# tub-rip/event_based_bos

Measured on AMD Instinct MI355X. Metric: Mevents/sec warped+IWE at 1280x720, higher is better.
Workload: dtype f32

## Files before the change

event_based_bos_amd/csrc/plan_lean.hip:

```cpp
#include <algorithm>
#include <type_traits>

#include "common.h"

namespace ebos {
namespace {

#ifdef EBOS_LEAN_STAMPS
__device__ unsigned long long g_lean_stamps[2][8192 * 8];
#define EBOS_LSTAMP(which, k)                                                                                     \
  do {                                                                                                            \
    if (threadIdx.x == 0 && blockIdx.x < 8192) g_lean_stamps[which][blockIdx.x * 8 + (k)] = wall_clock64();       \
  } while (0)
#else
#define EBOS_LSTAMP(which, k) \
  do {                        \
  } while (0)
#endif

constexpr int kChunk = 8192;
constexpr int kLeanBlock = 1024;
constexpr int kMaxBins = 8192;
constexpr int kSortBlock = 1024;
constexpr size_t kSortLds = 158 * 1024;

enum LeanSource { SRC_AOS_F32 = 0, SRC_AOS_F64 = 1, SRC_RAW32 = 2, SRC_RAW64 = 3 };

struct LeanIn {
  const void* events;
  const int16_t* col;
  const int16_t* row;
  const void* t;
  double ticks_per_second;
};

struct Ev {
  float x, y;
  double t;
};

template <int SRC>
__device__ __forceinline__ Ev read_event(const LeanIn& in, int64_t i) {
  Ev e;
  if (SRC == SRC_AOS_F32) {
    const float4 v = reinterpret_cast<const float4*>(in.events)[i];
    e.x = v.x, e.y = v.y, e.t = (double)v.z;
  } else if (SRC == SRC_AOS_F64) {
    const double2 a = reinterpret_cast<const double2*>(in.events)[2 * i];
    const double tt = reinterpret_cast<const double*>(in.events)[4 * i + 2];
    e.x = (float)a.x, e.y = (float)a.y, e.t = tt;
  } else {
    e.x = (float)in.row[i];
    e.y = (float)in.col[i];
    e.t = SRC == SRC_RAW32 ? (double)static_cast<const int32_t*>(in.t)[i] : (double)static_cast<const int64_t*>(in.t)[i];
  }
  return e;
}

struct LeanGeom {
  int H, W, th, tw, tiles_x, n_tiles, sub, n_bins;
  int chunk;
  unsigned m_th, m_tw;
};
__device__ __forceinline__ int div_small(int v, int d, unsigned m) { return m ? (int)__umulhi((unsigned)v, m) : v / d; }

__device__ __forceinline__ int event_bin(const LeanGeom& g, float x, float y, unsigned& pix, bool& fractional) {
  fractional = false;
  if (!(x > -1e9f && x < 1e9f && y > -1e9f && y < 1e9f)) return -1;
  const int r = (int)x, c = (int)y;
  if (r < 0 || r >= g.H || c < 0 || c >= g.W) return -1;
  fractional = (x != (float)r) || (y != (float)c) || x < 0.f || y < 0.f;
  const int ty = div_small(r, g.th, g.m_th), tx = div_small(c, g.tw, g.m_tw);
  const int rl = r - ty * g.th, cl = c - tx * g.tw;
  pix = ((unsigned)rl << 8) | (unsigned)cl;
  return (ty * g.tiles_x + tx) * g.sub + div_small(rl * g.sub, g.th, g.m_th);
}
__device__ __forceinline__ int band_row0(const LeanGeom& g, int s) { return (s * g.th + g.sub - 1) / g.sub; }

__device__ __forceinline__ unsigned long long ordered(double v) {
  const unsigned long long b = (unsigned long long)__double_as_longlong(v);
  return (b >> 63) ? ~b : (b | 0x8000000000000000ull);
}
__device__ __forceinline__ double unordered(unsigned long long u) {
  const unsigned long long b = (u >> 63) ? (u & 0x7fffffffffffffffull) : ~u;
  return __longlong_as_double((long long)b);
}

constexpr int kTabShift = 14;
constexpr unsigned kTabMask = (1u << kTabShift) - 1u;

struct ChunkPartial {
  double lo, hi;
  int bad, frac;
};

struct LeanScratch {
  unsigned* tab;
  int32_t* bin_base;
  unsigned long long* tm;
  unsigned* ticket;
  ChunkPartial* partial;
  uint16_t* stage_px;
  void* stage_t;
};

template <int SRC> struct StageT { typedef unsigned type; };
template <> struct StageT<SRC_AOS_F64> { typedef unsigned long long type; };
template <> struct StageT<SRC_RAW64> { typedef unsigned long long type; };

template <int SRC>
__device__ __forceinline__ typename StageT<SRC>::type read_stamp(const LeanIn& in, int64_t i, float& x, float& y, double& t) {
  if (SRC == SRC_AOS_F32) {
    const float4 v = reinterpret_cast<const float4*>(in.events)[i];
    x = v.x, y = v.y, t = (double)v.z;
    return (typename StageT<SRC>::type)__float_as_uint(v.z);
  } else if (SRC == SRC_AOS_F64) {
    const double2 a = reinterpret_cast<const double2*>(in.events)[2 * i];
    const double tt = reinterpret_cast<const double*>(in.events)[4 * i + 2];
    x = (float)a.x, y = (float)a.y, t = tt;
    return (typename StageT<SRC>::type)__double_as_longlong(tt);
  } else if (SRC == SRC_RAW32) {
    x = (float)in.row[i], y = (float)in.col[i];
    const int32_t k = static_cast<const int32_t*>(in.t)[i];
    t = (double)k;
    return (typename StageT<SRC>::type)(unsigned)k;
  } else {
    x = (float)in.row[i], y = (float)in.col[i];
    const int64_t k = static_cast<const int64_t*>(in.t)[i];
    t = (double)k;
    return (typename StageT<SRC>::type)k;
  }
}
__device__ __forceinline__ double stamp_seconds(int src, const void* stage_t, int64_t i, double ticks_per_second) {
  switch (src) {
    case SRC_AOS_F32: return (double)static_cast<const float*>(stage_t)[i];
    case SRC_AOS_F64: return static_cast<const double*>(stage_t)[i];
    case SRC_RAW32: return (double)static_cast<const int32_t*>(stage_t)[i] / ticks_per_second;
    default: return (double)static_cast<const int64_t*>(stage_t)[i] / ticks_per_second;
  }
}

__device__ __forceinline__ int32_t block_exclusive_scan(int32_t v, int32_t* s_wave , int32_t& total) {
  const int lane = threadIdx.x & (kWave - 1), wid = threadIdx.x / kWave;
  int32_t inc = v;
#pragma unroll
  for (int off = 1; off < kWave; off <<= 1) {
    const int32_t o = __shfl_up(inc, off, kWave);
    if (lane >= off) inc += o;
  }
  if (lane == kWave - 1) s_wave[wid] = inc;
  __syncthreads();
  int32_t wave_off = 0, tot = 0;
#pragma unroll
  for (int k = 0; k < kLeanBlock / kWave; ++k) {
    const int32_t w = s_wave[k];
    wave_off += k < wid ? w : 0;
    tot += w;
  }
  total = tot;
  __syncthreads();
  return wave_off + inc - v;
}

struct StageOne {
  LeanIn in;
  int64_t n;
  LeanGeom g;
  LeanScratch sc;
  struct View {
    LeanIn in;
    int64_t n;
    LeanGeom g;
    LeanScratch sc;
    __device__ __forceinline__ unsigned index() const { return blockIdx.x; }
    __device__ __forceinline__ unsigned count() const { return gridDim.x; }
  };
  __device__ __forceinline__ View view() const { return View{in, n, g, sc}; }
};

template <int SRC, typename Args>
__global__ void __launch_bounds__(kLeanBlock, 8)
lean_stage_kernel(Args args) {
  const typename Args::View v = args.view();
  const LeanIn in = v.in;
  const int64_t n = v.n;
  const LeanGeom g = v.g;
  const LeanScratch sc = v.sc;
  typedef typename StageT<SRC>::type stamp_t;
  extern __shared__ int32_t s_mem[];
  int32_t* s_hist = s_mem;
  stamp_t* s_t = reinterpret_cast<stamp_t*>(s_mem + ((g.n_bins + 1) & ~1));
  uint16_t* s_px = reinterpret_cast<uint16_t*>(s_t + g.chunk);
  __shared__ int32_t s_wave[kLeanBlock / kWave + 1];
  EBOS_LSTAMP(0, 0);
  for (int b = threadIdx.x; b < g.n_bins; b += kLeanBlock) s_hist[b] = 0;
  if (v.index() == 0 && threadIdx.x == 0) *sc.ticket = 0u;
  __syncthreads();
  constexpr int kPer = kChunk / kLeanBlock;
  const int64_t base = (int64_t)v.index() * g.chunk;
  const int64_t chunk_end = min(n, base + g.chunk);
  double lo = 1.0e308 * 10.0, hi = -1.0e308 * 10.0;
  int bad = 0, frac = 0;
  int bin_of[kPer];
  unsigned pix[kPer];
  stamp_t stamp[kPer];
#pragma unroll
  for (int k = 0; k < kPer; ++k) {
    if (k == kPer / 2) asm volatile("" ::: "memory");
    const int64_t i = base + k * kLeanBlock + threadIdx.x;
    bin_of[k] = -1;
    if (i < chunk_end) {
      float x, y;
      double t;
      stamp[k] = read_stamp<SRC>(in, i, x, y, t);
      lo = t < lo ? t : lo;
      hi = t > hi ? t : hi;
      bool fr;
      const int b = event_bin(g, x, y, pix[k], fr);
      bin_of[k] = b;
      bad += b < 0;
      frac += fr;
    }
  }
  EBOS_LSTAMP(0, 1);
#pragma unroll
  for (int k = 0; k < kPer; ++k)
    if (bin_of[k] >= 0) bin_of[k] |= atomicAdd(&s_hist[bin_of[k]], 1) << 13;
  __syncthreads();
  EBOS_LSTAMP(0, 2);
  const int per = (g.n_bins + kLeanBlock - 1) / kLeanBlock;
  const int b0 = threadIdx.x * per;
  int32_t mine = 0;
  for (int j = 0; j < per; ++j) mine += b0 + j < g.n_bins ? s_hist[b0 + j] : 0;
  int32_t kept;
  int32_t run = block_exclusive_scan(mine, s_wave, kept);
  for (int j = 0; j < per; ++j)
    if (b0 + j < g.n_bins) {
      const int32_t c = s_hist[b0 + j];
      s_hist[b0 + j] = run;
      sc.tab[(int64_t)(b0 + j) * v.count() + v.index()] = (unsigned)run | ((unsigned)c << kTabShift);
      run += c;
    }
  __syncthreads();
  EBOS_LSTAMP(0, 3);
#pragma unroll
  for (int k = 0; k < kPer; ++k)
    if (bin_of[k] >= 0) {
      const int pos = s_hist[bin_of[k] & 8191] + (bin_of[k] >> 13);
      s_t[pos] = stamp[k];
      s_px[pos] = (uint16_t)pix[k];
    }
  __syncthreads();
  EBOS_LSTAMP(0, 4);
  stamp_t* out_t = static_cast<stamp_t*>(sc.stage_t) + base;
  for (int i = threadIdx.x; i < kept; i += kLeanBlock) out_t[i] = s_t[i];
  unsigned* out_px = reinterpret_cast<unsigned*>(sc.stage_px + base);
  const unsigned* s_px2 = reinterpret_cast<const unsigned*>(s_px);
  for (int i = threadIdx.x; i < (kept + 1) / 2; i += kLeanBlock) out_px[i] = s_px2[i];
  __shared__ double s_lo[kLeanBlock / kWave], s_hi[kLeanBlock / kWave];
  __shared__ int s_bad[kLeanBlock / kWave], s_frac[kLeanBlock / kWave];
  lo = wave_min(lo);
  hi = wave_max(hi);
  bad = wave_sum(bad);
  frac = wave_sum(frac);
  if ((threadIdx.x & (kWave - 1)) == 0) {
    s_lo[threadIdx.x / kWave] = lo;
    s_hi[threadIdx.x / kWave] = hi;
    s_bad[threadIdx.x / kWave] = bad;
    s_frac[threadIdx.x / kWave] = frac;
  }
  __syncthreads();
  if (threadIdx.x == 0) {
    for (int k = 1; k < kLeanBlock / kWave; ++k) {
      lo = s_lo[k] < lo ? s_lo[k] : lo;
      hi = s_hi[k] > hi ? s_hi[k] : hi;
      bad += s_bad[k];
      frac += s_frac[k];
    }
    sc.partial[v.index()] = ChunkPartial{lo, hi, bad, frac};
  }
  EBOS_LSTAMP(0, 5);
}

struct WholeGrid {
  __device__ __forceinline__ unsigned index() const { return blockIdx.x; }
  __device__ __forceinline__ unsigned count() const { return gridDim.x; }
};
struct GridPart {
  unsigned idx, cnt;
  __device__ __forceinline__ unsigned index() const { return idx; }
  __device__ __forceinline__ unsigned count() const { return cnt; }
};

__device__ __forceinline__ void lean_scan_bins_block(const LeanGeom& g, const LeanScratch& sc, int32_t* __restrict__ grp_offsets,
                                                     int32_t* __restrict__ key_offsets, int64_t n_keys, double ticks_per_second, int raw,
                                                     double* __restrict__ tminmax) {
  __shared__ int32_t s_wave[1024 / kWave];
  __shared__ int32_t s_carry;
  typedef __attribute__((address_space(1))) int32_t gi32_;
  auto total_of = [&](int b) { return __hip_atomic_load((gi32_*)(sc.bin_base + b), __ATOMIC_RELAXED, __HIP_MEMORY_SCOPE_AGENT); };
  const int lane = threadIdx.x & (kWave - 1), wid = threadIdx.x / kWave;
  auto scan = [&](int count, auto value, auto store) {
    if (threadIdx.x == 0) s_carry = 0;
    __syncthreads();
    for (int start = 0; start < count; start += 1024) {
      const int i = start + threadIdx.x;
      const int32_t v = i < count ? value(i) : 0;
      int32_t inc = v;
#pragma unroll
      for (int off = 1; off < kWave; off <<= 1) {
        const int32_t o = __shfl_up(inc, off, kWave);
        if (lane >= off) inc += o;
      }
      if (lane == kWave - 1) s_wave[wid] = inc;
      __syncthreads();
      int32_t wave_off = 0;
      for (int k = 0; k < wid; ++k) wave_off += s_wave[k];
      const int32_t carry = s_carry;
      if (i < count) store(i, carry + wave_off + inc - v);
      __syncthreads();
      if (threadIdx.x == 1023) s_carry = carry + wave_off + inc;
      __syncthreads();
    }
  };
  scan(g.n_tiles,
       [&](int t) {
         int32_t c = 0;
         for (int s = 0; s < g.sub; ++s) c += total_of(t * g.sub + s);
         return (c + 3) >> 2;
       },
       [&](int t, int32_t pre) { grp_offsets[t] = pre; });
  if (threadIdx.x == 0) grp_offsets[g.n_tiles] = s_carry;
  __syncthreads();
  scan(g.n_bins, [&](int b) { return total_of(b); }, [&](int b, int32_t pre) { sc.bin_base[b] = pre; });
  if (threadIdx.x == 0) {
    sc.bin_base[g.n_bins] = s_carry;
    key_offsets[n_keys] = s_carry;
    if (tminmax != nullptr) {
      const double lo = unordered(sc.tm[0]), hi = unordered(sc.tm[1]);
      tminmax[0] = raw ? lo / ticks_per_second : lo;
      tminmax[1] = raw ? hi / ticks_per_second : hi;
    }
  }
}

template <typename Grid>
__device__ __forceinline__ void lean_totals_body(const LeanGeom& g, int n_chunks, const LeanScratch& sc, int32_t* __restrict__ counts,
                                                 int32_t* __restrict__ grp_offsets, int32_t* __restrict__ key_offsets, int64_t n_keys,
                                                 double ticks_per_second, int raw, double* __restrict__ tminmax, const Grid grid) {
  __shared__ int s_is_last;
  {
    const int bin = grid.index() * (kLeanBlock / kWave) + (int)(threadIdx.x / kWave), lane = threadIdx.x & (kWave - 1);
    if (bin < g.n_bins) {
      const unsigned* __restrict__ row = sc.tab + (int64_t)bin * n_chunks;
      int32_t acc = 0;
      constexpr int kU = 4;
      for (int c = lane; c < n_chunks; c += kWave * kU) {
        unsigned v[kU];
#pragma unroll
        for (int u = 0; u < kU; ++u) v[u] = c + kWave * u < n_chunks ? row[c + kWave * u] : 0u;
#pragma unroll
        for (int u = 0; u < kU; ++u) acc += (int32_t)(v[u] >> kTabShift);
      }
      acc = wave_sum(acc);
      if (lane == 0) {
        typedef __attribute__((address_space(1))) int32_t gi32_;
        __hip_atomic_store((gi32_*)(sc.bin_base + bin), acc, __ATOMIC_RELAXED, __HIP_MEMORY_SCOPE_AGENT);
        asm volatile("s_waitcnt vmcnt(0)" ::: "memory");
      }
    }
  }
  if (grid.index() == 0) {
    double lo = 1.0e308 * 10.0, hi = -1.0e308 * 10.0;
    int bad = 0, frac = 0;
    for (int c = threadIdx.x; c < n_chunks; c += kLeanBlock) {
      const ChunkPartial p = sc.partial[c];
      lo = p.lo < lo ? p.lo : lo;
      hi = p.hi > hi ? p.hi : hi;
      bad += p.bad;
      frac += p.frac;
    }
    __shared__ double s_lo[kLeanBlock / kWave], s_hi[kLeanBlock / kWave];
    __shared__ int s_bad[kLeanBlock / kWave], s_frac[kLeanBlock / kWave];
    lo = wave_min(lo);
    hi = wave_max(hi);
    bad = wave_sum(bad);
    frac = wave_sum(frac);
    if ((threadIdx.x & (kWave - 1)) == 0) {
      s_lo[threadIdx.x / kWave] = lo;
      s_hi[threadIdx.x / kWave] = hi;
      s_bad[threadIdx.x / kWave] = bad;
      s_frac[threadIdx.x / kWave] = frac;
    }
    __syncthreads();
    if (threadIdx.x == 0) {
      for (int k = 1; k < kLeanBlock / kWave; ++k) {
        lo = s_lo[k] < lo ? s_lo[k] : lo;
        hi = s_hi[k] > hi ? s_hi[k] : hi;
        bad += s_bad[k];
        frac += s_frac[k];
      }
      typedef __attribute__((address_space(1))) unsigned long long gu64_;
      __hip_atomic_store((gu64_*)&sc.tm[0], lo <= hi ? ordered(lo) : ~0ull, __ATOMIC_RELAXED, __HIP_MEMORY_SCOPE_AGENT);
      __hip_atomic_store((gu64_*)&sc.tm[1], lo <= hi ? ordered(hi) : 0ull, __ATOMIC_RELAXED, __HIP_MEMORY_SCOPE_AGENT);
      counts[0] = bad;
      counts[1] = frac;
    }
  }
  __syncthreads();
  if (threadIdx.x == 0) {
    typedef __attribute__((address_space(1))) unsigned gu32_;
    asm volatile("s_waitcnt vmcnt(0)" ::: "memory");
    const unsigned n_wg = grid.count();
    s_is_last = __hip_atomic_fetch_add((gu32_*)sc.ticket, 1u, __ATOMIC_RELAXED, __HIP_MEMORY_SCOPE_AGENT) == n_wg - 1u;
  }
  __syncthreads();
  if (!s_is_last) return;
  if (threadIdx.x == 0) {
    typedef __attribute__((address_space(1))) unsigned long long gu64_;
    sc.tm[0] = __hip_atomic_load((gu64_*)&sc.tm[0], __ATOMIC_RELAXED, __HIP_MEMORY_SCOPE_AGENT);
    sc.tm[1] = __hip_atomic_load((gu64_*)&sc.tm[1], __ATOMIC_RELAXED, __HIP_MEMORY_SCOPE_AGENT);
  }
  __syncthreads();
  lean_scan_bins_block(g, sc, grp_offsets, key_offsets, n_keys, ticks_per_second, raw, tminmax);
}

__global__ void __launch_bounds__(kLeanBlock)
lean_totals_kernel(LeanGeom g, int n_chunks, LeanScratch sc, int32_t* __restrict__ counts, int32_t* __restrict__ grp_offsets,
                   int32_t* __restrict__ key_offsets, int64_t n_keys, double ticks_per_second, int raw, double* __restrict__ tminmax) {
  lean_totals_body(g, n_chunks, sc, counts, grp_offsets, key_offsets, n_keys, ticks_per_second, raw, tminmax, WholeGrid{});
}

struct LeanTime {
  int src, ref_mode, normalize_t;
  double ref_fraction, ticks_per_second;
};

template <int STRIDE>
__device__ __forceinline__ int row_xor(int v) {
  static_assert(STRIDE == 1 || STRIDE == 2 || STRIDE == 4 || STRIDE == 8, "row_xor: 1, 2, 4 or 8");
  if (STRIDE == 1) return __builtin_amdgcn_update_dpp(0, v, 0xB1, 0xf, 0xf, false);
  if (STRIDE == 2) return __builtin_amdgcn_update_dpp(0, v, 0x4E, 0xf, 0xf, false);
  if (STRIDE == 8) return __builtin_amdgcn_update_dpp(0, v, 0x128, 0xf, 0xf, false);
  const int m = __builtin_amdgcn_update_dpp(0, v, 0x141, 0xf, 0xf, false);
  return __builtin_amdgcn_update_dpp(0, m, 0x1B, 0xf, 0xf, false);
}
template <int SIZE, int STRIDE>
__device__ __forceinline__ int bitonic16_step(int key, int sub16) {
  const int other = row_xor<STRIDE>(key);
  const bool up = (sub16 & SIZE) == 0;
  const bool low = (sub16 & STRIDE) == 0;
  const int mn = min(key, other), mx = max(key, other);
  return (low == up) ? mn : mx;
}
__device__ __forceinline__ int bitonic16(int key, int sub16, int longest) {
  key = bitonic16_step<2, 1>(key, sub16);
  if (longest > 2) {
    key = bitonic16_step<4, 2>(key, sub16);
    key = bitonic16_step<4, 1>(key, sub16);
  }
  if (longest > 4) {
    key = bitonic16_step<8, 4>(key, sub16);
    key = bitonic16_step<8, 2>(key, sub16);
    key = bitonic16_step<8, 1>(key, sub16);
  }
  if (longest > 8) {
    key = bitonic16_step<16, 8>(key, sub16);
    key = bitonic16_step<16, 4>(key, sub16);
    key = bitonic16_step<16, 2>(key, sub16);
    key = bitonic16_step<16, 1>(key, sub16);
  }
  return key;
}

__device__ __forceinline__ int sort_key(float d) {
  const int b = __float_as_int(d);
  return b ^ ((b >> 31) & 0x7fffffff);
}

struct LeanRec {
  unsigned pix;
  unsigned long long stamp;
};
struct LeanClock {
  double ref, inv_period, tps;
  bool raw, wide;
  __device__ __forceinline__ LeanClock(const LeanScratch& sc, const LeanTime& tc) {
    raw = tc.src == SRC_RAW32 || tc.src == SRC_RAW64;
    wide = tc.src == SRC_AOS_F64 || tc.src == SRC_RAW64;
    tps = tc.ticks_per_second;
    double tmin = unordered(sc.tm[0]), tmax = unordered(sc.tm[1]);
    if (raw) {
      tmin = tmin / tps;
      tmax = tmax / tps;
    } else if (tc.src == SRC_AOS_F32) {
      tmin = (double)(float)tmin;
      tmax = (double)(float)tmax;
    }
    if (tc.ref_mode == EBOS_REF_FIRST) ref = tmin;
    else if (tc.ref_mode == EBOS_REF_LAST) ref = tmax;
    else ref = tmin + (tmax - tmin) * tc.ref_fraction;
    inv_period = tc.normalize_t ? 1.0 / (tmax - tmin) : 1.0;
  }
  __device__ __forceinline__ float dt(const LeanRec& r) const {
    const double t8 = raw ? (double)(long long)r.stamp / tps : __longlong_as_double((long long)r.stamp);
    const double t4 = raw ? (double)(int32_t)(unsigned)r.stamp / tps : (double)__uint_as_float((unsigned)r.stamp);
    return (float)(((wide ? t8 : t4) - ref) * inv_period);
  }
};

template <bool POS, int BLOCK, typename Load, typename Use>
__device__ __forceinline__ void lean_gather(const LeanScratch& sc, const LeanGeom& g, int bin, int n_chunks, int32_t* s_arrived, Load&& load,
                                            Use&& use) {
  typedef decltype(load((int64_t)0)) payload_t;
  const int lane = threadIdx.x & (kWave - 1);
  const unsigned* __restrict__ my_tab = sc.tab + (int64_t)bin * n_chunks;
  unsigned e_next = (int)threadIdx.x < n_chunks ? my_tab[threadIdx.x] : 0u;
  for (int blk = 0; blk < n_chunks; blk += BLOCK) {
    const unsigned e = e_next;
    const int c_next = blk + BLOCK + threadIdx.x;
    e_next = c_next < n_chunks ? my_tab[c_next] : 0u;
    const int my_cnt = (int)(e >> kTabShift), my_off = (int)(e & kTabMask);
    if (__ballot(my_cnt > 0) == 0ull) continue;
    int my_pos = 0;
    if (POS) {
      int inc = my_cnt;
#pragma unroll
      for (int off = 1; off < kWave; off <<= 1) {
        const int o = __shfl_up(inc, off, kWave);
        if (lane >= off) inc += o;
      }
      int wave_base = 0;
      if (lane == kWave - 1) wave_base = atomicAdd(s_arrived, inc);
      my_pos = __shfl(wave_base, kWave - 1, kWave) + inc - my_cnt;
    }
    const int64_t wave_chunk0 = blk + (threadIdx.x & ~(kWave - 1));
    const int i0 = lane & 7;
    for (int base = 0; __ballot(my_cnt > base) != 0ull; base += 16) {
      payload_t v[16];
      int cnt[8], pos[8];
#pragma unroll
      for (int k = 0; k < 8; ++k) {
        const int r = 8 * k + (lane >> 3);
        cnt[k] = __shfl(my_cnt, r, kWave) - base;
        pos[k] = (POS ? __shfl(my_pos, r, kWave) : 0) + base;
        const int off = __shfl(my_off, r, kWave);
        const int64_t src = cnt[k] > 0 ? (wave_chunk0 + r) * g.chunk + off + base : 0;
        v[2 * k] = load(src + min(i0, max(cnt[k] - 1, 0)));
        v[2 * k + 1] = load(src + min(i0 + 8, max(cnt[k] - 1, 0)));
      }
#pragma unroll
      for (int k = 0; k < 8; ++k) {
        if (i0 < cnt[k]) use(v[2 * k], pos[k] + i0);
        if (i0 + 8 < cnt[k]) use(v[2 * k + 1], pos[k] + i0 + 8);
      }
    }
  }
}

__device__ __forceinline__ void lean_bin_sort_body(const LeanGeom& g, const LeanScratch& sc, const int32_t* __restrict__ grp_offsets,
                                                   int32_t* __restrict__ key_offsets, uint16_t* __restrict__ cpix, float* __restrict__ cdt,
                                                   int pix_cap, int sort_cap, int n_chunks, const LeanTime& tc) {
  extern __shared__ int32_t s_raw[];
  int32_t* s_cnt = s_raw;
  int32_t* s_cur = s_raw + pix_cap;
  float* a_dt = reinterpret_cast<float*>(s_raw + 2 * pix_cap);
  float* s_dt = a_dt + sort_cap;
  uint16_t* a_px = reinterpret_cast<uint16_t*>(s_dt + sort_cap);
  uint16_t* s_px = a_px + sort_cap;
  __shared__ int32_t s_wave[kSortBlock / kWave];
  __shared__ int32_t s_arrived;
  const int per_xcd = (g.n_bins + 7) / 8;
  const int bin = (int)(blockIdx.x & 7u) * per_xcd + (int)(blockIdx.x >> 3);
  if (bin >= g.n_bins) return;
  const int tile = bin / g.sub, band = bin - tile * g.sub;
  const int r0 = band_row0(g, band), r1 = band_row0(g, band + 1);
  const int n_pix = (r1 - r0) * g.tw;
  const int32_t seg0 = sc.bin_base[bin], seg1 = sc.bin_base[bin + 1], len = seg1 - seg0;
  const int64_t first_key = (int64_t)tile * g.th * g.tw + (int64_t)r0 * g.tw;
  const int32_t tile_first = sc.bin_base[tile * g.sub];
  const int64_t out0 = (int64_t)grp_offsets[tile] * 4 + (seg0 - tile_first);
  EBOS_LSTAMP(1, 0);
  for (int i = threadIdx.x; i < n_pix; i += kSortBlock) s_cnt[i] = 0;
  if (threadIdx.x == 0) s_arrived = 0;
  __syncthreads();
  const bool staged = len <= sort_cap;
  const int lane = threadIdx.x & (kWave - 1);
  const LeanClock clock(sc, tc);
  typedef LeanRec Rec;
  auto dt_of = [&](const Rec& r) { return clock.dt(r); };
  const bool wide = clock.wide;
  auto load8 = [&](int64_t i) { return Rec{(unsigned)sc.stage_px[i], static_cast<const unsigned long long*>(sc.stage_t)[i]}; };
  auto load4 = [&](int64_t i) { return Rec{(unsigned)sc.stage_px[i], (unsigned long long)static_cast<const unsigned*>(sc.stage_t)[i]}; };
  auto for_each_staged = [&](auto with_pos, auto&& load, auto&& use) {
    lean_gather<decltype(with_pos)::value, kSortBlock>(sc, g, bin, n_chunks, &s_arrived, load, use);
  };
  if (staged) {
    auto arrive = [&](const Rec& r, int at) {
      a_px[at] = (uint16_t)r.pix;
      a_dt[at] = dt_of(r);
      atomicAdd(&s_cnt[((int)(r.pix >> 8) - r0) * g.tw + (int)(r.pix & 255u)], 1);
    };
    if (wide) for_each_staged(std::true_type{}, load8, arrive);
    else for_each_staged(std::true_type{}, load4, arrive);
  } else {
    for_each_staged(std::false_type{}, [&](int64_t i) { return (unsigned)sc.stage_px[i]; },
                    [&](unsigned pix, int) { atomicAdd(&s_cnt[((int)(pix >> 8) - r0) * g.tw + (int)(pix & 255u)], 1); });
  }
  __syncthreads();
  EBOS_LSTAMP(1, 1);
  const int wid = threadIdx.x / kWave;
  {
    const int per = (n_pix + kSortBlock - 1) / kSortBlock, p0 = threadIdx.x * per;
    int32_t mine = 0;
    for (int j = 0; j < per; ++j) mine += p0 + j < n_pix ? s_cnt[p0 + j] : 0;
    int32_t inc = mine;
#pragma unroll
    for (int off = 1; off < kWave; off <<= 1) {
      const int32_t o = __shfl_up(inc, off, kWave);
      if (lane >= off) inc += o;
    }
    if (lane == kWave - 1) s_wave[wid] = inc;
    __syncthreads();
    int32_t run = inc - mine;
    for (int k = 0; k < wid; ++k) run += s_wave[k];
    for (int j = 0; j < per; ++j)
      if (p0 + j < n_pix) {
        const int32_t c = s_cnt[p0 + j];
        s_cnt[p0 + j] = run;
        s_cur[p0 + j] = run;
        key_offsets[first_key + p0 + j] = seg0 + run;
        run += c;
      }
    __syncthreads();
  }
  EBOS_LSTAMP(1, 2);
  if (staged) {
    for (int i = threadIdx.x; i < len; i += kSortBlock) {
      const unsigned pix = (unsigned)a_px[i];
      const int32_t pos = atomicAdd(&s_cur[((int)(pix >> 8) - r0) * g.tw + (int)(pix & 255u)], 1);
      s_px[pos] = (uint16_t)pix;
      s_dt[pos] = a_dt[i];
    }
  }
  __syncthreads();
  EBOS_LSTAMP(1, 3);
  if (!staged) {
    s_dt = a_dt;
    s_px = a_px;
    sort_cap *= 2;
  }
  constexpr int kLeanCanon = 1024, kHotList = 32;
  __shared__ int32_t s_hot[kHotList];
  __shared__ int32_t s_nhot, s_nlong;
  auto run_end = [&](int pi) { return pi + 1 < n_pix ? s_cnt[pi + 1] : len; };
  int p_lo = 0;
  while (p_lo < n_pix) {
    const int c0 = s_cnt[p_lo];
    int p_hi = n_pix;
    if (!staged) {
      int lo = p_lo, hi = n_pix;
      while (lo < hi) {
        const int mid = lo + (hi - lo) / 2;
        if (run_end(mid) - c0 <= sort_cap) lo = mid + 1;
        else hi = mid;
      }
      p_hi = lo;
    }
    const bool direct = p_hi == p_lo;
    if (direct) p_hi = p_lo + 1;
    const int c1 = p_hi < n_pix ? s_cnt[p_hi] : len, m = c1 - c0;
    if (threadIdx.x == 0) s_nhot = 0, s_nlong = 0;
    if (!staged) {
      __syncthreads();
      auto keep = [&](const Rec& r, int) {
        const int pi = ((int)(r.pix >> 8) - r0) * g.tw + (int)(r.pix & 255u);
        if (pi >= p_lo && pi < p_hi) {
          const int32_t pos = atomicAdd(&s_cur[pi], 1);
          if (direct) {
            cpix[out0 + pos] = (uint16_t)r.pix;
            cdt[out0 + pos] = dt_of(r);
          } else {
            s_px[pos - c0] = (uint16_t)r.pix;
            s_dt[pos - c0] = dt_of(r);
          }
        }
      };
      if (wide) for_each_staged(std::false_type{}, load8, keep);
      else for_each_staged(std::false_type{}, load4, keep);
      if (direct) {
        p_lo = p_hi;
        continue;
      }
    }
    __syncthreads();
    for (int pi = p_lo + threadIdx.x; pi < p_hi; pi += kSortBlock)
      if (run_end(pi) - s_cnt[pi] > kLeanCanon) {
        const int k = atomicAdd(&s_nhot, 1);
        if (k < kHotList) s_hot[k] = pi;
      }
    __syncthreads();
    EBOS_LSTAMP(1, 5);
    for (int i = threadIdx.x; i < m; i += kSortBlock) cpix[out0 + c0 + i] = s_px[i];
    const int n_hot = min(s_nhot, kHotList);
    for (int h = 0; h < n_hot; ++h) {
      const int pi = s_hot[h];
      const int rb = s_cnt[pi] - c0, L = run_end(pi) - c0 - rb;
      float* v = s_dt + rb;
      int n2 = 1;
      while (n2 < L) n2 <<= 1;
      for (int size = 2; size <= n2; size <<= 1) {
        for (int stride = size >> 1; stride > 0; stride >>= 1) {
          for (int t = threadIdx.x; t < n2 / 2; t += kSortBlock) {
            const int blk = t / stride, off = t - blk * stride, lo = blk * 2 * stride + off;
            const int hi = stride == (size >> 1) ? blk * 2 * stride + (2 * stride - 1 - off) : lo + stride;
            if (hi < L) {
              const float x = v[lo], y = v[hi];
              if (sort_key(x) > sort_key(y)) v[lo] = y, v[hi] = x;
            }
          }
          __syncthreads();
        }
      }
    }
    EBOS_LSTAMP(1, 6);
    const bool sparse = m < 4 * (p_hi - p_lo);
    if (sparse) {
      for (int i = threadIdx.x; i < m; i += kSortBlock) {
        const unsigned px = (unsigned)s_px[i];
        const int pi = ((int)(px >> 8) - r0) * g.tw + (int)(px & 255u);
        const int rb = s_cnt[pi] - c0, re = run_end(pi) - c0;
        const float d = s_dt[i];
        int slot = i;
        if (re - rb > 1 && re - rb <= kLeanCanon) {
          const int kd = sort_key(d);
          int rank = 0;
          for (int j = rb; j < re; ++j) {
            const int kj = sort_key(s_dt[j]);
            rank += (kj < kd || (kj == kd && j < i)) ? 1 : 0;
          }
          slot = rb + rank;
        }
        cdt[out0 + c0 + slot] = d;
      }
    } else {
      const int sub16 = lane & 15;
      for (int p0 = p_lo; p0 < p_hi; p0 += kSortBlock / 16) {
        const int pi = p0 + (threadIdx.x >> 4);
        const bool live = pi < p_hi;
        const int rb = live ? s_cnt[pi] - c0 : 0, L = live ? run_end(pi) - c0 - rb : 0;
        const bool small = L <= 16;
        int key = small && sub16 < L ? sort_key(s_dt[rb + sub16]) : 0x7fffffff;
        const int longest = __ballot(small && L > 8) != 0ull ? 16 : (__ballot(small && L > 4) != 0ull ? 8 : (__ballot(small && L > 2) != 0ull ? 4 : (__ballot(small && L > 1) != 0ull ? 2 : 1)));
        if (longest > 1) key = bitonic16(key, sub16, longest);
        if (small && sub16 < L) cdt[out0 + c0 + rb + sub16] = __int_as_float(key ^ ((key >> 31) & 0x7fffffff));
        if (!small && sub16 == 0) s_cur[atomicAdd(&s_nlong, 1)] = pi;
      }
    }
    __syncthreads();
    if (!sparse) {
      const int n_long = s_nlong, sub32 = lane & 31;
      for (int q = threadIdx.x >> 5; q < n_long; q += kSortBlock / 32) {
        const int pi = s_cur[q];
        const int rb = s_cnt[pi] - c0, L = run_end(pi) - c0 - rb;
        for (int e = sub32; e < L; e += 32) {
          const float d = s_dt[rb + e];
          int slot = e;
          if (L <= kLeanCanon) {
            const int kd = sort_key(d);
            int rank = 0;
            for (int j = 0; j < L; ++j) {
              const int kj = sort_key(s_dt[rb + j]);
              rank += (kj < kd || (kj == kd && j < e)) ? 1 : 0;
            }
            slot = rank;
          }
          cdt[out0 + c0 + rb + slot] = d;
        }
      }
    }
    EBOS_LSTAMP(1, 7);
    __syncthreads();
    p_lo = p_hi;
  }
  EBOS_LSTAMP(1, 4);
  if (band == g.sub - 1) {
    const int64_t end = (int64_t)grp_offsets[tile + 1] * 4;
    for (int64_t o = out0 + len + threadIdx.x; o < end; o += kSortBlock) {
      cpix[o] = 0;
      cdt[o] = __builtin_nanf("");
    }
  }
}

__global__ void __launch_bounds__(kSortBlock)
lean_bin_sort_kernel(LeanGeom g, LeanScratch sc, const int32_t* __restrict__ grp_offsets, int32_t* __restrict__ key_offsets,
                     uint16_t* __restrict__ cpix, float* __restrict__ cdt, int pix_cap, int sort_cap, int n_chunks, LeanTime tc) {
  lean_bin_sort_body(g, sc, grp_offsets, key_offsets, cpix, cdt, pix_cap, sort_cap, n_chunks, tc);
}

struct LeanSections {
  size_t off_base, off_tm, off_partial, off_px, off_t, total;
};
__host__ __device__ __forceinline__ LeanSections lean_sections(int n_bins, int n_chunks, int chunk) {
  auto align = [](size_t v) { return (v + 255) & ~(size_t)255; };
  LeanSections S;
  S.off_base = align((size_t)n_bins * n_chunks * 4);
  S.off_tm = S.off_base + align((size_t)(n_bins + 1) * 4);
  S.off_partial = S.off_tm + 256;
  S.off_px = S.off_partial + align((size_t)n_chunks * sizeof(ChunkPartial));
  S.off_t = S.off_px + align((size_t)n_chunks * chunk * 2);
  S.total = S.off_t + align((size_t)n_chunks * chunk * 8);
  return S;
}
__host__ __device__ __forceinline__ LeanScratch lean_scratch_at(char* base, const LeanSections& S) {
  return LeanScratch{reinterpret_cast<unsigned*>(base), reinterpret_cast<int32_t*>(base + S.off_base),
                     reinterpret_cast<unsigned long long*>(base + S.off_tm), reinterpret_cast<unsigned*>(base + S.off_tm + 64),
                     reinterpret_cast<ChunkPartial*>(base + S.off_partial), reinterpret_cast<uint16_t*>(base + S.off_px),
                     base + S.off_t};
}
__host__ __device__ __forceinline__ void lean_sort_caps(int th, int tw, int sub, int& pix_cap, int& sort_cap) {
  pix_cap = ((th + sub - 1) / sub + 1) * tw;
  const long long room = (long long)kSortLds - (long long)pix_cap * 8;
  sort_cap = room > 0 ? (int)(room / 12) & ~1 : 0;
}

struct LeanLayout {
  int n_chunks, chunk, sub, n_bins, pix_cap, sort_cap;
  size_t off_base, off_tm, off_partial, off_px, off_t, total;
};

inline LeanLayout lean_layout(int64_t n, int H, int W, int th, int tw) {
  LeanLayout L;
  const int n_tiles = ((H + th - 1) / th) * ((W + tw - 1) / tw);
  constexpr int64_t kResident = 512;
  int64_t c = (n + kChunk - 1) / kChunk;
  if (c > kResident) c = (c + kResident - 1) / kResident * kResident;
  else c = std::min<int64_t>(kResident, std::max<int64_t>(1, (n + kLeanBlock - 1) / kLeanBlock));
  L.chunk = (int)(((std::max<int64_t>(n, 1) + c - 1) / c + 7) & ~(int64_t)7);
  L.n_chunks = (int)((std::max<int64_t>(n, 1) + L.chunk - 1) / L.chunk);
  constexpr double kBinFill = 3.3;
  for (int sub = 1;; sub *= 2) {
    if (sub > th) sub = th;
    L.sub = sub;
    lean_sort_caps(th, tw, sub, L.pix_cap, L.sort_cap);
    if (sub == th || ((double)n / ((double)n_tiles * sub) <= kBinFill * L.sort_cap)) break;
  }
  L.n_bins = n_tiles * L.sub;
  const LeanSections S = lean_sections(L.n_bins, L.n_chunks, L.chunk);
  L.off_base = S.off_base, L.off_tm = S.off_tm, L.off_partial = S.off_partial, L.off_px = S.off_px, L.off_t = S.off_t, L.total = S.total;
  return L;
}

struct LeanWin {
  int64_t begin;
  int64_t scratch_off;
  int64_t slot_off;
  int32_t n;
  int32_t chunk0;
  int32_t n_chunks, chunk, sub;
  int32_t reserved;
};
constexpr int kLeanBatch = 64;
struct LeanBatch {
  LeanWin w[kLeanBatch];
};
static_assert(sizeof(LeanBatch) <= 3072, "the batch travels in the kernel argument segment");
struct LeanBatchOut {
  int32_t* key_offsets;
  int32_t* grp_offsets;
  uint16_t* cpix;
  float* cdt;
  int32_t* counts;
  double* tminmax;
  char* scratch;
  int64_t key_stride, grp_stride;
  int first;
};
__device__ __forceinline__ LeanIn lean_window_in(const LeanIn& in, int wide, int64_t begin) {
  return LeanIn{nullptr, in.col + begin, in.row + begin,
                wide ? static_cast<const void*>(static_cast<const int64_t*>(in.t) + begin)
                     : static_cast<const void*>(static_cast<const int32_t*>(in.t) + begin),
                in.ticks_per_second};
}
__device__ __forceinline__ LeanGeom lean_window_geom(LeanGeom g, const LeanWin& w) {
  g.sub = w.sub, g.n_bins = g.n_tiles * w.sub, g.chunk = w.chunk;
  return g;
}
__device__ __forceinline__ LeanScratch lean_window_scratch(const LeanBatchOut& o, const LeanGeom& g, const LeanWin& w) {
  return lean_scratch_at(o.scratch + w.scratch_off, lean_sections(g.n_bins, w.n_chunks, w.chunk));
}

struct StageMany {
  LeanBatch b;
  int n_windows, wide;
  LeanIn in;
  LeanGeom g0;
  LeanBatchOut o;
  struct View {
    LeanIn in;
    int64_t n;
    LeanGeom g;
    LeanScratch sc;
    unsigned idx, cnt;
    __device__ __forceinline__ unsigned index() const { return idx; }
    __device__ __forceinline__ unsigned count() const { return cnt; }
  };
  __device__ __forceinline__ View view() const {
    int lo = 0, hi = n_windows - 1;
    while (lo < hi) {
      const int mid = (lo + hi + 1) >> 1;
      if ((unsigned)b.w[mid].chunk0 <= blockIdx.x) lo = mid;
      else hi = mid - 1;
    }
    const LeanWin w = b.w[lo];
    const LeanGeom g = lean_window_geom(g0, w);
    return View{lean_window_in(in, wide, w.begin), (int64_t)w.n, g, lean_window_scratch(o, g, w), blockIdx.x - (unsigned)w.chunk0,
                (unsigned)w.n_chunks};
  }
};
static_assert(sizeof(StageMany) <= 3584, "the batch travels in the kernel argument segment");

__global__ void __launch_bounds__(kLeanBlock)
lean_totals_batch_kernel(LeanBatch b, LeanGeom g0, LeanBatchOut o, int64_t n_keys, double ticks_per_second) {
  const LeanWin w = b.w[blockIdx.y];
  const LeanGeom g = lean_window_geom(g0, w);
  const unsigned n_wg = (unsigned)((g.n_bins + kLeanBlock / kWave - 1) / (kLeanBlock / kWave));
  if (blockIdx.x >= n_wg) return;
  const int64_t wi = o.first + (int64_t)blockIdx.y;
  lean_totals_body(g, w.n_chunks, lean_window_scratch(o, g, w), o.counts + 2 * wi, o.grp_offsets + wi * o.grp_stride,
                   o.key_offsets + wi * o.key_stride, n_keys, ticks_per_second, 1, o.tminmax ? o.tminmax + 2 * wi : nullptr,
                   GridPart{blockIdx.x, n_wg});
}

__global__ void __launch_bounds__(kSortBlock)
lean_bin_sort_batch_kernel(LeanBatch b, LeanGeom g0, LeanBatchOut o, LeanTime tc) {
  const LeanWin w = b.w[blockIdx.y];
  const LeanGeom g = lean_window_geom(g0, w);
  if (blockIdx.x >= 8u * (unsigned)((g.n_bins + 7) / 8)) return;
  const int64_t wi = o.first + (int64_t)blockIdx.y;
  int pix_cap, sort_cap;
  lean_sort_caps(g.th, g.tw, g.sub, pix_cap, sort_cap);
  lean_bin_sort_body(g, lean_window_scratch(o, g, w), o.grp_offsets + wi * o.grp_stride, o.key_offsets + wi * o.key_stride,
                     o.cpix + w.slot_off, o.cdt + w.slot_off, pix_cap, sort_cap, w.n_chunks, tc);
}

}
}

extern "C" {

#ifdef EBOS_LEAN_STAMPS
int ebos_debug_read_lean_stamps(unsigned long long* host, int count) {
  return (int)hipMemcpyFromSymbol(host, HIP_SYMBOL(ebos::g_lean_stamps), sizeof(unsigned long long) * count);
}
#endif

size_t ebos_plan_lean_scratch_bytes(int64_t n, int H, int W, int tile_h, int tile_w) {
  if (n < 0 || H <= 0 || W <= 0 || tile_h <= 0 || tile_w <= 0) return 0;
  return ebos::lean_layout(n, H, W, tile_h, tile_w).total;
}

int ebos_plan_lean(int source, const void* events, const int16_t* col, const int16_t* row, const void* t, double ticks_per_second,
                   int64_t n, int ref_mode, double ref_fraction, int normalize_t, int H, int W, int tile_h, int tile_w,
                   int32_t* key_offsets, int32_t* grp_offsets, uint16_t* cpix, float* cdt, int64_t capacity_slots, int32_t* counts,
                   double* tminmax, void* scratch, size_t scratch_bytes, ebos_stream_t stream) {
  using namespace ebos;
  EBOS_REQUIRE(source >= 0 && source <= 3, "ebos_plan_lean: source must be 0 (f32 [n,4]), 1 (f64 [n,4]), 2 (raw, int32 t), 3 (raw, int64 t)");
  EBOS_REQUIRE(n >= 1 && n < (int64_t)1 << 31, "ebos_plan_lean: 1 <= n < 2^31 (got %lld)", (long long)n);
  EBOS_REQUIRE(H > 0 && W > 0 && tile_h > 0 && tile_w > 0 && tile_h <= 256 && tile_w <= 256, "ebos_plan_lean: bad sizes (tiles up to 256 x 256)");
  EBOS_REQUIRE(ref_mode >= 0 && ref_mode <= 2, "ebos_plan_lean: ref_mode must be FIRST / LAST / FRACTION");
  EBOS_REQUIRE(source <= 1 ? events != nullptr : (col && row && t && ticks_per_second > 0.0), "ebos_plan_lean: NULL event buffer");
  EBOS_REQUIRE(key_offsets && grp_offsets && cpix && cdt && counts && scratch, "ebos_plan_lean: NULL output / scratch");
  const int tiles_y = (H + tile_h - 1) / tile_h, tiles_x = (W + tile_w - 1) / tile_w, n_tiles = tiles_y * tiles_x;
  const int64_t n_keys = (int64_t)n_tiles * tile_h * tile_w;
  const LeanLayout L = lean_layout(n, H, W, tile_h, tile_w);
  if (L.n_bins > kMaxBins || L.sort_cap < 64) {
    set_error("ebos_plan_lean: %d bins / %d pixels per band exceed what this build sorts in LDS", L.n_bins, L.pix_cap);
    return EBOS_ERR_UNSUPPORTED;
  }
  if (scratch_bytes < L.total) {
    set_error("ebos_plan_lean: scratch too small (%zu < %zu)", scratch_bytes, L.total);
    return EBOS_ERR_SCRATCH;
  }
  if (capacity_slots < n + 3 * (int64_t)n_tiles + 4) {
    set_error("ebos_plan_lean: capacity %lld < n + 3 tiles + 4 = %lld", (long long)capacity_slots, (long long)(n + 3 * (int64_t)n_tiles + 4));
    return EBOS_ERR_SCRATCH;
  }
  hipStream_t s = as_stream(stream);
  char* base = reinterpret_cast<char*>(scratch);
  const LeanScratch sc = lean_scratch_at(base, lean_sections(L.n_bins, L.n_chunks, L.chunk));
  const bool small = H <= 65536 && W <= 65536;
  const LeanGeom g{H, W, tile_h, tile_w, tiles_x, n_tiles, L.sub, L.n_bins, L.chunk,
                   small ? (unsigned)(0x100000000ull / (unsigned)tile_h) + 1u : 0u, small ? (unsigned)(0x100000000ull / (unsigned)tile_w) + 1u : 0u};
  const LeanIn in{events, col, row, t, ticks_per_second};
  const size_t stamp_bytes = (source == SRC_AOS_F64 || source == SRC_RAW64) ? 8 : 4;
  const size_t lds_stage = (size_t)((L.n_bins + 1) & ~1) * 4 + (size_t)L.chunk * (stamp_bytes + 2);
  const size_t lds_sort = (size_t)(2 * L.pix_cap) * 4 + (size_t)L.sort_cap * 12;
  bool ok = hipFuncSetAttribute(reinterpret_cast<const void*>(lean_bin_sort_kernel), hipFuncAttributeMaxDynamicSharedMemorySize,
                                (int)kSortLds) == hipSuccess;
#define EBOS_LEAN_ATTR(SRC)                                                                                                  \
  ok = ok && hipFuncSetAttribute(reinterpret_cast<const void*>(lean_stage_kernel<SRC, StageOne>), hipFuncAttributeMaxDynamicSharedMemorySize, \
                                 (int)lds_stage) == hipSuccess
#define EBOS_LEAN(SRC)                                                                                                       \
  do {                                                                                                                       \
    EBOS_LEAN_ATTR(SRC);                                                                                                     \
    if (ok) lean_stage_kernel<SRC, StageOne><<<dim3(L.n_chunks), dim3(kLeanBlock), lds_stage, s>>>(StageOne{in, n, g, sc});  \
  } while (0)
  if (source == SRC_AOS_F32) EBOS_LEAN(SRC_AOS_F32);
  else if (source == SRC_AOS_F64) EBOS_LEAN(SRC_AOS_F64);
  else if (source == SRC_RAW32) EBOS_LEAN(SRC_RAW32);
  else EBOS_LEAN(SRC_RAW64);
#undef EBOS_LEAN
#undef EBOS_LEAN_ATTR
  if (!ok) {
    set_error("ebos_plan_lean: cannot reserve LDS for the staging pass / the bin sort");
    return EBOS_ERR_LAUNCH;
  }
  lean_totals_kernel<<<dim3((L.n_bins + kLeanBlock / kWave - 1) / (kLeanBlock / kWave)), dim3(kLeanBlock), 0, s>>>(g, L.n_chunks, sc, counts, grp_offsets, key_offsets, n_keys,
                                                                                     ticks_per_second, source >= SRC_RAW32, tminmax);
  const LeanTime tc{source, ref_mode, normalize_t, ref_fraction, ticks_per_second};
  lean_bin_sort_kernel<<<dim3(8 * ((L.n_bins + 7) / 8)), dim3(kSortBlock), lds_sort, s>>>(g, sc, grp_offsets, key_offsets, cpix, cdt, L.pix_cap, L.sort_cap,
                                                                          L.n_chunks, tc);
  EBOS_CHECK_LAUNCH("ebos_plan_lean");
  return EBOS_OK;
}

size_t ebos_plan_lean_batch_scratch_bytes(const int64_t* ranges, int n_windows, int H, int W, int tile_h, int tile_w) {
  if (ranges == nullptr || n_windows < 1 || H <= 0 || W <= 0 || tile_h <= 0 || tile_w <= 0) return 0;
  size_t total = 0;
  for (int w = 0; w < n_windows; ++w) {
    const int64_t n = ranges[2 * w + 1] - ranges[2 * w];
    if (n < 0) return 0;
    total += ebos::lean_layout(n, H, W, tile_h, tile_w).total;
  }
  return total;
}

int ebos_plan_lean_batch(const int16_t* col, const int16_t* row, const void* t, int t_is_64, double ticks_per_second, int64_t n_total,
                         const int64_t* ranges, int n_windows, int ref_mode, double ref_fraction, int normalize_t, int H, int W,
                         int tile_h, int tile_w, int32_t* key_offsets, int64_t key_stride, int32_t* grp_offsets, int64_t grp_stride,
                         uint16_t* cpix, float* cdt, const int64_t* slot_offsets, int32_t* counts, double* tminmax, void* scratch,
                         size_t scratch_bytes, ebos_stream_t stream) {
  using namespace ebos;
  EBOS_REQUIRE(n_windows >= 1 && n_total >= 0 && ranges && slot_offsets, "ebos_plan_lean_batch: no windows / NULL host table");
  EBOS_REQUIRE(H > 0 && W > 0 && tile_h > 0 && tile_w > 0 && tile_h <= 256 && tile_w <= 256, "ebos_plan_lean_batch: bad sizes (tiles up to 256 x 256)");
  EBOS_REQUIRE(ref_mode >= 0 && ref_mode <= 2, "ebos_plan_lean_batch: ref_mode must be FIRST / LAST / FRACTION");
  EBOS_REQUIRE(col && row && t && ticks_per_second > 0.0, "ebos_plan_lean_batch: NULL event columns");
  EBOS_REQUIRE(key_offsets && grp_offsets && cpix && cdt && counts && scratch, "ebos_plan_lean_batch: NULL output / scratch");
  const int tiles_y = (H + tile_h - 1) / tile_h, tiles_x = (W + tile_w - 1) / tile_w, n_tiles = tiles_y * tiles_x;
  const int64_t n_keys = (int64_t)n_tiles * tile_h * tile_w;
  EBOS_REQUIRE(key_stride >= n_keys + 1 && grp_stride >= n_tiles + 1, "ebos_plan_lean_batch: strides shorter than a window's arrays");
  size_t need = 0;
  for (int w = 0; w < n_windows; ++w) {
    const int64_t b = ranges[2 * w], e = ranges[2 * w + 1], n = e - b;
    EBOS_REQUIRE(b >= 0 && e >= b && e <= n_total && n < (int64_t)1 << 31, "ebos_plan_lean_batch: window %d = [%lld, %lld) outside the %lld events",
                 w, (long long)b, (long long)e, (long long)n_total);
    EBOS_REQUIRE(slot_offsets[w] >= 0 && slot_offsets[w] % 8 == 0 && slot_offsets[w + 1] - slot_offsets[w] >= n + 3 * (int64_t)n_tiles + 4,
                 "ebos_plan_lean_batch: window %d: slots must start on a multiple of 8 and hold n + 3 tiles + 4", w);
    const LeanLayout L = lean_layout(n, H, W, tile_h, tile_w);
    if (L.n_bins > kMaxBins || L.sort_cap < 64) {
      set_error("ebos_plan_lean_batch: %d bins / %d pixels per band exceed what this build sorts in LDS", L.n_bins, L.pix_cap);
      return EBOS_ERR_UNSUPPORTED;
    }
    need += L.total;
  }
  if (scratch_bytes < need) {
    set_error("ebos_plan_lean_batch: scratch too small (%zu < %zu)", scratch_bytes, need);
    return EBOS_ERR_SCRATCH;
  }
  hipStream_t s = as_stream(stream);
  const int source = t_is_64 ? SRC_RAW64 : SRC_RAW32;
  const bool small = H <= 65536 && W <= 65536;
  const LeanGeom g0{H, W, tile_h, tile_w, tiles_x, n_tiles, 1, n_tiles, 8,
                    small ? (unsigned)(0x100000000ull / (unsigned)tile_h) + 1u : 0u, small ? (unsigned)(0x100000000ull / (unsigned)tile_w) + 1u : 0u};
  const LeanIn in{nullptr, col, row, t, ticks_per_second};
  const LeanTime tc{source, ref_mode, normalize_t, ref_fraction, ticks_per_second};
  const size_t stamp_bytes = t_is_64 ? 8 : 4;
  bool ok = hipFuncSetAttribute(reinterpret_cast<const void*>(lean_bin_sort_batch_kernel), hipFuncAttributeMaxDynamicSharedMemorySize,
                                (int)kSortLds) == hipSuccess;
  size_t scratch_off = 0;
  for (int first = 0; first < n_windows && ok; first += kLeanBatch) {
    const int nw = std::min(kLeanBatch, n_windows - first);
    LeanBatch b{};
    int chunks = 0, max_bins = 0;
    size_t lds_stage = 0, lds_sort = 0;
    for (int k = 0; k < nw; ++k) {
      const int w = first + k;
      const int64_t n = ranges[2 * w + 1] - ranges[2 * w];
      const LeanLayout L = lean_layout(n, H, W, tile_h, tile_w);
      b.w[k] = LeanWin{ranges[2 * w], (int64_t)scratch_off, slot_offsets[w], (int32_t)n, chunks, L.n_chunks, L.chunk, L.sub, 0};
      scratch_off += L.total;
      chunks += L.n_chunks;
      max_bins = std::max(max_bins, L.n_bins);
      lds_stage = std::max(lds_stage, (size_t)((L.n_bins + 1) & ~1) * 4 + (size_t)L.chunk * (stamp_bytes + 2));
      lds_sort = std::max(lds_sort, (size_t)(2 * L.pix_cap) * 4 + (size_t)L.sort_cap * 12);
    }
    const LeanBatchOut o{key_offsets, grp_offsets, cpix, cdt, counts, tminmax, reinterpret_cast<char*>(scratch), key_stride, grp_stride, first};
    const StageMany many{b, nw, t_is_64 ? 1 : 0, in, g0, o};
    if (t_is_64) {
      ok = hipFuncSetAttribute(reinterpret_cast<const void*>(lean_stage_kernel<SRC_RAW64, StageMany>), hipFuncAttributeMaxDynamicSharedMemorySize,
                               (int)lds_stage) == hipSuccess;
      if (ok) lean_stage_kernel<SRC_RAW64, StageMany><<<dim3(chunks), dim3(kLeanBlock), lds_stage, s>>>(many);
    } else {
      ok = hipFuncSetAttribute(reinterpret_cast<const void*>(lean_stage_kernel<SRC_RAW32, StageMany>), hipFuncAttributeMaxDynamicSharedMemorySize,
                               (int)lds_stage) == hipSuccess;
      if (ok) lean_stage_kernel<SRC_RAW32, StageMany><<<dim3(chunks), dim3(kLeanBlock), lds_stage, s>>>(many);
    }
    if (!ok) break;
    lean_totals_batch_kernel<<<dim3((max_bins + kLeanBlock / kWave - 1) / (kLeanBlock / kWave), nw), dim3(kLeanBlock), 0, s>>>(
        b, g0, o, n_keys, ticks_per_second);
    lean_bin_sort_batch_kernel<<<dim3(8 * ((max_bins + 7) / 8), nw), dim3(kSortBlock), lds_sort, s>>>(b, g0, o, tc);
  }
  if (!ok) {
    set_error("ebos_plan_lean_batch: cannot reserve LDS for the staging pass / the bin sort");
    return EBOS_ERR_LAUNCH;
  }
  EBOS_CHECK_LAUNCH("ebos_plan_lean_batch");
  return EBOS_OK;
}

}
```

event_based_bos_amd/event_plan.py:

```python
from __future__ import annotations

import ctypes as C
from dataclasses import dataclass, fields
from typing import List, NamedTuple, Optional, Sequence, Tuple, Union

import torch
from torch.utils import _pytree

from . import _hip, ops
from ._hip import check, ptr, stream_ptr

DEFAULT_TILE = (64, 64)
DEFAULT_HALO = 32


def choose_tile(image_size: Tuple[int, int], halo: int = DEFAULT_HALO, n_cu: int = 256) -> Tuple[int, int]:
    H, W = image_size
    best, best_cost = DEFAULT_TILE, None
    for th, tw, hl in _hip.slab_configs():
        if hl != halo:
            continue
        tiles = ((H + th - 1) // th) * ((W + tw - 1) // tw)
        rounds = (tiles + n_cu - 1) // n_cu
        cost = rounds * (th * tw + 0.15 * (th + 2 * hl) * (tw + 2 * hl))
        if best_cost is None or cost < best_cost:
            best, best_cost = (th, tw), cost
    return best


def parse_direction(direction: Union[str, float]) -> Tuple[int, float]:
    import numpy as np

    if type(direction) is float:
        return _hip.REF_FRACTION, direction
    if direction == "first":
        return _hip.REF_FIRST, 0.0
    if direction == "middle":
        return _hip.REF_FRACTION, 0.5
    if direction == "last":
        return _hip.REF_LAST, 1.0
    if direction == "random":
        return _hip.REF_FRACTION, float(np.random.uniform(low=0.0, high=1.0))
    if direction == "before":
        return _hip.REF_FRACTION, -1.0
    if direction == "after":
        return _hip.REF_FRACTION, 2.0
    raise ValueError(f"direction argument should be first, middle, last. Or float. {direction}")


def dt_bound_for(direction: Union[str, float], normalize_t: bool) -> Optional[float]:
    if not normalize_t:
        return None
    _, frac = parse_direction(direction)
    return max(abs(frac), abs(1.0 - frac))


def ref_fraction_for(direction: Union[str, float]) -> Optional[float]:
    if type(direction) is str and direction == "random":
        return None
    return float(parse_direction(direction)[1])


def resolve_halo(plan: "EventPlan", halo) -> int:
    if halo != "auto":
        return int(halo)
    biggest = max((hl for th, tw, hl in _hip.slab_configs() if (th, tw) == tuple(plan.tile)), default=None)
    if biggest is None:
        raise ValueError(f"no tile-private kernels are built for tile {plan.tile}")
    if plan.dt_bound is None:
        return biggest
    return int(_hip.load_library().ebos_halo_auto(biggest, float(plan.dt_bound)))


def _norm_halo(plan: "EventPlan", halo):
    if halo is None or halo != "auto":
        return halo
    return resolve_halo(plan, halo) if plan.binned else None


def _max_halo(halo: int) -> int:
    return halo if halo >= 0 else (-halo) & 255


_N_CU = {}


def _n_cu(device: torch.device) -> int:
    idx = device.index if device.index is not None else torch.cuda.current_device()
    if idx not in _N_CU:
        _N_CU[idx] = torch.cuda.get_device_properties(idx).multi_processor_count
    return _N_CU[idx]


PART_FIXED_EVENTS = 8192


def part_fixed_events(n_events: int, n_tiles: int, n_cu: int) -> int:
    if 2 * n_tiles <= n_cu:
        return PART_FIXED_EVENTS
    return int(min(65536, max(PART_FIXED_EVENTS, 6.5e10 / max(int(n_events), 1))))


class PlanBatchLayout(NamedTuple):
    n_tiles: int
    n_keys: int
    key_stride: int
    grp_stride: int
    part_stride: int
    capacities: Tuple[int, ...]
    slot_offsets: Tuple[int, ...]


PLAN_BATCH_ALIGN = 64


def plan_batch_layout(lengths: Sequence[int], image_size: Tuple[int, int], tile: Tuple[int, int]) -> PlanBatchLayout:
    H, W = int(image_size[0]), int(image_size[1])
    th, tw = int(tile[0]), int(tile[1])
    if H <= 0 or W <= 0 or th <= 0 or tw <= 0:
        raise ValueError("plan_batch_layout: image and tile sizes must be positive")
    n_tiles = ((H + th - 1) // th) * ((W + tw - 1) // tw)
    n_keys = n_tiles * th * tw
    up = lambda v: (v + PLAN_BATCH_ALIGN - 1) // PLAN_BATCH_ALIGN * PLAN_BATCH_ALIGN
    caps, offs = [], [0]
    for n in lengths:
        n = int(n)
        if n < 0:
            raise ValueError("plan_batch_layout: a window cannot hold a negative number of events")
        caps.append(n + 3 * n_tiles + 8)
        offs.append(offs[-1] + up(caps[-1]))
    return PlanBatchLayout(n_tiles, n_keys, up(n_keys + 1), up(n_tiles + 1), up(5 * n_tiles + 1), tuple(caps), tuple(offs))


@dataclass
class EventPlan:

    x: Optional[torch.Tensor]
    y: Optional[torch.Tensor]
    dt: Optional[torch.Tensor]
    p: Optional[torch.Tensor]
    image_size: Tuple[int, int]
    n: int
    n_input: int
    tile: Optional[Tuple[int, int]] = None
    key_offsets: Optional[torch.Tensor] = None
    perm: Optional[torch.Tensor] = None
    n_dropped: int = 0
    grp_offsets: Optional[torch.Tensor] = None
    cpix: Optional[torch.Tensor] = None
    cdt: Optional[torch.Tensor] = None
    part_table: Optional[torch.Tensor] = None
    dt_bound: Optional[float] = None
    bins: Optional[torch.Tensor] = None
    time_bin: Optional[int] = None
    ref_fraction: Optional[float] = None
    normalized_t: Optional[bool] = None

    @property
    def binned(self) -> bool:
        return self.key_offsets is not None

    @property
    def device(self) -> torch.device:
        return (self.x if self.x is not None else self.key_offsets).device

    @property
    def lean(self) -> bool:
        return self.x is None

    @property
    def compact(self) -> bool:
        return self.cpix is not None

    def clear_cache(self) -> None:
        for k in ("_workspaces", "_jobs", "_sweep_lanes", "_multiref_dts", "_canonical_stack"):
            self.__dict__.pop(k, None)

    def resolve_splits(self, splits: Optional[int]) -> int:
        if splits is not None:
            return int(splits)
        if self.part_table is None:
            return 1
        used = self.__dict__.get("_parts_used")
        n_tiles = (self.part_table.numel() - 1) // 5
        return 1 if used is not None and used <= n_tiles else 0

    LOOP_ADAPTIVE_MIN_EXCESS = 48_000

    def resolve_loop_splits(self, splits: Optional[int]) -> int:
        s = self.resolve_splits(splits)
        fullest = self.__dict__.get("_fullest_tile")
        if splits is None and s == 0 and fullest is not None:
            n_tiles = (self.part_table.numel() - 1) // 5
            if fullest - self.n / max(n_tiles, 1) < self.LOOP_ADAPTIVE_MIN_EXCESS:
                return 1
        return s

    def _compact_ptrs(self):
        return (ptr(self.grp_offsets), ptr(self.cpix), ptr(self.cdt)) if self.compact else (None, None, None)

    @property
    def fractional(self) -> bool:
        return bool(self.__dict__.get("_frac_pending")) or self.__dict__.get("_frac") is not None

    def _frac_ptrs(self, query: bool = False):
        if query and self.__dict__.get("_frac") is None:
            return (1,) * 5
        return tuple(ptr(t) for t in self.frac_compact)

    def record_stream(self, stream: torch.cuda.Stream) -> None:
        for t in (*(getattr(self, f.name) for f in fields(self)), *(self.__dict__.get("_frac") or ())):
            if isinstance(t, torch.Tensor):
                t.record_stream(stream)

    @property
    def frac_compact(self):
        d = self.__dict__
        if d.get("_frac") is None and d.get("_frac_pending"):
            lib = _hip.require_gpu()
            dev = self.x.device
            H, W = self.image_size
            th, tw = self.tile
            n_tiles = ((H + th - 1) // th) * ((W + tw - 1) // tw)
            cap = self.n + 3 * n_tiles + 8
            f_grp = torch.empty(n_tiles + 1, dtype=torch.int32, device=dev)
            f_pix = torch.zeros(cap, dtype=torch.int16, device=dev)
            f_dt = torch.full((cap,), float("nan"), dtype=torch.float32, device=dev)
            f_x, f_y = torch.zeros(cap, dtype=torch.float32, device=dev), torch.zeros(cap, dtype=torch.float32, device=dev)
            with _hip.on_device(dev):
                check(lib.ebos_plan_compact_frac_f32(ptr(self.x), ptr(self.y), ptr(self.dt), ptr(self.key_offsets), self.n, H, W, th, tw,
                                                     ptr(f_grp), ptr(f_pix), ptr(f_dt), ptr(f_x), ptr(f_y), cap, stream_ptr()),
                      "ebos_plan_compact_frac")
            d["_frac"], d["_frac_pending"] = (f_grp, f_pix, f_dt, f_x, f_y), False
        return d.get("_frac")

    @staticmethod
    def build(events: torch.Tensor, image_size: Tuple[int, int], direction: Union[str, float] = "first",
              normalize_t: bool = True, tile: Optional[Tuple[int, int]] = DEFAULT_TILE, emit: str = "full",
              deferred: bool = False, time_bin: Optional[int] = None) -> "EventPlan":
        if emit not in ("full", "compact"):
            raise ValueError("emit must be 'full' or 'compact'")
        if time_bin is not None:
            time_bin = ops.check_time_bins(time_bin)
            if emit != "full" or deferred:
                raise NotImplementedError('EventPlan.build: time_bin needs the SoA events and the permutation of emit="full" with '
                                          "deferred=False (a lean, compact or deferred plan keeps neither)")
        if isinstance(tile, str):
            if tile != "auto":
                raise ValueError("tile must be a (tile_h, tile_w) pair, None or 'auto'")
            tile = choose_tile(image_size)
        lib = _hip.require_gpu()
        if events.dim() != 2 or events.shape[-1] != 4:
            raise ValueError(f"EventPlan.build expects un-batched events [n,4], got {tuple(events.shape)}")
        if not events.is_cuda:
            raise _hip.HipUnavailableError("EventPlan.build: events must be on the GPU")
        events = events.contiguous()
        if emit == "compact" and deferred:
            raise ValueError("EventPlan.build: emit='compact' with deferred=True needs integer source coordinates by construction: "
                             "use build_raw (sensor columns), or deferred=False")
        if emit == "compact" and tile is not None and events.shape[0] > 0:
            lean = _build_lean(0 if events.dtype == torch.float32 else 1, events, None, image_size, direction, normalize_t, tile,
                               1.0, deferred)
            if lean is not None:
                return lean
        H, W = int(image_size[0]), int(image_size[1])
        n = events.shape[0]
        ref_mode, frac = parse_direction(direction)
        dev = events.device
        tmm = ops.time_range(events[None])
        x, y, dt, p = (torch.empty(n, dtype=torch.float32, device=dev) for _ in range(4))
        with _hip.on_device(dev):
            fn = getattr(lib, "ebos_events_to_soa_" + _hip.suffix(events.dtype))
            check(fn(ptr(events), ptr(tmm), ref_mode, frac, int(normalize_t), n, ptr(x), ptr(y), ptr(dt), ptr(p),
                     stream_ptr()), "ebos_events_to_soa")
        plan = EventPlan(x, y, dt, p, (H, W), n, n, dt_bound=dt_bound_for(direction, normalize_t),
                         ref_fraction=ref_fraction_for(direction), normalized_t=bool(normalize_t))
        if time_bin is not None:
            plan.bins, plan.time_bin = ops.time_bins(events[None], time_bin, tmm)[0], time_bin
        if tile is not None:
            plan = plan.bin(tile)
        return plan

    @staticmethod
    def build_raw(col: torch.Tensor, row: torch.Tensor, t: torch.Tensor, pol: torch.Tensor, image_size: Tuple[int, int],
                  direction: Union[str, float] = "first", normalize_t: bool = True,
                  tile: Optional[Tuple[int, int]] = DEFAULT_TILE, ticks_per_second: float = 1e6,
                  deferred: bool = False, emit: str = "full", time_bin: Optional[int] = None) -> "EventPlan":
        if time_bin is not None:
            raise NotImplementedError('EventPlan.build_raw: a time-aware plan (time_bin) is built from the event array: '
                                      'EventPlan.build(events, ..., emit="full", time_bin=T)')
        if isinstance(tile, str):
            if tile != "auto":
                raise ValueError("tile must be a (tile_h, tile_w) pair, None or 'auto'")
            tile = choose_tile(image_size)
        lib = _hip.require_gpu()
        n = int(t.shape[0])
        for name, v, dts in (("col", col, (torch.int16,)), ("row", row, (torch.int16,)), ("t", t, (torch.int32, torch.int64)),
                             ("pol", pol, (torch.bool, torch.uint8))):
            if v.dim() != 1 or v.shape[0] != n or v.dtype not in dts:
                raise ValueError(f"EventPlan.build_raw: {name} must be a 1-D tensor of {n} elements, dtype in {dts}; "
                                 f"got {tuple(v.shape)} {v.dtype}")
            if not v.is_cuda:
                raise _hip.HipUnavailableError(f"EventPlan.build_raw: {name} must be on the GPU")
        if n == 0:
            raise IndexError("EventPlan.build_raw: empty window")
# ... 319 lines not shown
                       pad: Tuple[int, int] = (0, 0), halo: Optional[int] = DEFAULT_HALO,
                       splits: Optional[int] = None, sign: float = 1.0, _eager_checked: bool = False) -> torch.Tensor:
        halo = _norm_halo(self, halo)
        if cost not in ("image_variance", "gradient_magnitude"):
            raise KeyError(f"unknown contrast cost {cost!r}")
        if cost == "image_variance" or _slab_ok(self, halo):
            pad2, splits = (int(pad[0]), int(pad[1])), self.resolve_splits(splits)
            if _eager_checked or _eager_ok(self, flow, halo):
                sign = float(sign)
                spec = -1.0 if sign == 1.0 else sign
                out, d_flow = _run_dense_job(_dense_job(self, pad2, halo, splits, bool(omit_boundary)), flow, True, cost, spec)
                return _EagerLoss.wrap(out[1] if sign != 1.0 else out[0], flow, d_flow, sign, applied=spec)
            v = _FusedVarianceDense.apply(flow, self, pad2, bool(omit_boundary), halo, splits, cost)
            return v if sign == 1.0 else v * sign
        v = ops.gradient_magnitude(self.iwe_dense(flow, pad=pad, halo=halo, splits=splits), omit_boundary)
        return v if sign == 1.0 else v * sign

    def iwe_dense_multi(self, flow: torch.Tensor, directions, pad: Tuple[int, int] = (0, 0), halo=DEFAULT_HALO,
                        splits: Optional[int] = None, fused: Optional[bool] = None) -> torch.Tensor:
        job = _multiref_job(self, directions, pad, halo, splits, fused, "iwe_dense_multi")
        if job.fused == "slab":
            return _MultiRefSlabIwe.apply(flow, self, job)
        return _MultiRefIwe.apply(flow, self, job)

    def contrast_dense_multi(self, flow: torch.Tensor, directions, cost: str = "image_variance", omit_boundary: bool = False,
                             pad: Tuple[int, int] = (0, 0), halo=DEFAULT_HALO, splits: Optional[int] = None,
                             fused: Optional[bool] = None) -> torch.Tensor:
        if cost not in ("image_variance", "gradient_magnitude"):
            raise KeyError(f"unknown contrast cost {cost!r}")
        job = _multiref_job(self, directions, pad, halo, splits, fused, "contrast_dense_multi")
        if job.fused == "slab":
            if cost == "image_variance":
                return _MultiRefSlabVariance.apply(flow, self, job, bool(omit_boundary))
            return ops.gradient_magnitude(_MultiRefSlabIwe.apply(flow, self, job), omit_boundary).mean()
        if cost == "image_variance":
            return _MultiRefVariance.apply(flow, self, job, bool(omit_boundary))
        return ops.gradient_magnitude(_MultiRefIwe.apply(flow, self, job), omit_boundary).mean()

    def variance_multi_value_and_grad(self, flow: torch.Tensor, directions, omit_boundary: bool = False, pad: Tuple[int, int] = (0, 0),
                                      halo=DEFAULT_HALO, splits: Optional[int] = None) -> Tuple[torch.Tensor, torch.Tensor]:
        job = _multiref_job(self, directions, pad, halo, splits, "slab", "variance_multi_value_and_grad")
        flow32 = _check_flow(self, flow)
        K = len(job.shifts)
        iwes, variances, moments = _launch_multiref_slab_fwd(self, flow32, job, 1, bool(omit_boundary))
        upstream = torch.full((1,), 1.0 / K, dtype=torch.float32, device=self.device)
        d_flow = _launch_multiref_slab_bwd(self, flow32, job, iwes, None, int(bool(omit_boundary)), moments, upstream)
        return variances.mean(), d_flow

    def iwe_voxel(self, voxel: torch.Tensor, pad: Tuple[int, int] = (0, 0), weight: Optional[torch.Tensor] = None,
                  halo: Optional[int] = DEFAULT_HALO, splits: Optional[int] = None) -> torch.Tensor:
        return _FusedIweVoxel.apply(voxel, weight, self, (int(pad[0]), int(pad[1])), _voxel_halo(self, halo), self.resolve_splits(splits))

    def contrast_voxel(self, voxel: torch.Tensor, cost: str = "image_variance", omit_boundary: bool = False,
                       pad: Tuple[int, int] = (0, 0), halo: Optional[int] = DEFAULT_HALO,
                       splits: Optional[int] = None) -> torch.Tensor:
        if cost not in ("image_variance", "gradient_magnitude"):
            raise KeyError(f"unknown contrast cost {cost!r}")
        pad2, halo, splits = (int(pad[0]), int(pad[1])), _voxel_halo(self, halo), self.resolve_splits(splits)
        if cost == "image_variance":
            return _FusedVarianceVoxel.apply(voxel, self, pad2, bool(omit_boundary), halo, splits)
        return ops.gradient_magnitude(_FusedIweVoxel.apply(voxel, None, self, pad2, halo, splits), omit_boundary)

    def variance_voxel_value_and_grad(self, voxel: torch.Tensor, omit_boundary: bool = False, pad: Tuple[int, int] = (0, 0),
                                      halo="auto", upstream: float = 1.0,
                                      out: Optional[torch.Tensor] = None) -> Tuple[torch.Tensor, torch.Tensor]:
        lib = _hip.require_gpu()
        vox32 = _check_voxel(self, voxel)
        if not self.binned:
            raise NotImplementedError("variance_voxel_value_and_grad walks the runs of a binned plan: build it with a tile "
                                      "(contrast_voxel serves an un-binned one)")
        _refuse_deferred(self, "variance_voxel_value_and_grad")
        pad2 = (int(pad[0]), int(pad[1]))
        H, W = self.image_size
        T = int(vox32.shape[0])
        dev = self.device
        if out is None:
            out = torch.empty((T, 2, H, W), dtype=torch.float32, device=dev)
        elif tuple(out.shape) != (T, 2, H, W) or out.dtype != torch.float32 or out.device != dev or not out.is_contiguous():
            raise ValueError(f"out must be a contiguous float32 tensor of shape {(T, 2, H, W)} on {dev}")
        iwe = _launch_iwe_voxel(self, vox32, None, pad2, _voxel_halo(self, halo), self.resolve_splits(None))
        h, w = iwe.shape
        value = torch.empty(1, dtype=torch.float32, device=dev)
        moments = torch.empty((1, 2), dtype=torch.float64, device=dev)
        affine = torch.empty(2, dtype=torch.float32, device=dev)
        up = torch.full((1,), float(upstream), dtype=torch.float32, device=dev)
        nbytes = int(lib.ebos_cost_scratch_bytes(1))
        scratch = torch.empty(nbytes, dtype=torch.uint8, device=dev)
        with _hip.on_device(dev):
            check(lib.ebos_image_variance_f32(ptr(iwe), 1, h, w, int(bool(omit_boundary)), ptr(value), ptr(moments), ptr(scratch), nbytes,
                                              stream_ptr()), "ebos_image_variance")
            check(lib.ebos_image_variance_affine_f32(ptr(moments), ptr(up), 1, ptr(affine), stream_ptr()), "ebos_image_variance_affine")
            check(lib.ebos_iwe_voxel_owner_bwd_f32(ptr(self.x), ptr(self.y), ptr(self.dt), None, ptr(self.bins), ptr(self.key_offsets),
                                                   self.n, ptr(vox32), T, H, W, self.tile[0], self.tile[1], pad2[0], pad2[1], ptr(iwe),
                                                   ptr(affine), int(bool(omit_boundary)), ptr(out), stream_ptr()),
                  "ebos_iwe_voxel_owner_bwd")
        return value, out

    def iwe_voxel_multi(self, voxel: torch.Tensor, directions, pad: Tuple[int, int] = (0, 0), halo: Optional[int] = DEFAULT_HALO,
                        splits: Optional[int] = None) -> torch.Tensor:
        job = _voxel_multi_job(self, directions, pad, halo, splits, "iwe_voxel_multi")
        return _MultiRefIweVoxel.apply(voxel, self, job)

    def contrast_voxel_multi(self, voxel: torch.Tensor, directions, cost: str = "image_variance", omit_boundary: bool = False,
                             pad: Tuple[int, int] = (0, 0), halo: Optional[int] = DEFAULT_HALO,
                             splits: Optional[int] = None) -> torch.Tensor:
        if cost not in ("image_variance", "gradient_magnitude"):
            raise KeyError(f"unknown contrast cost {cost!r}")
        job = _voxel_multi_job(self, directions, pad, halo, splits, "contrast_voxel_multi")
        if cost == "image_variance":
            return _MultiRefVarianceVoxel.apply(voxel, self, job, bool(omit_boundary))
        return ops.gradient_magnitude(_MultiRefIweVoxel.apply(voxel, self, job), omit_boundary).mean()

    def variance_voxel_multi_value_and_grad(self, voxel: torch.Tensor, directions, omit_boundary: bool = False,
                                            pad: Tuple[int, int] = (0, 0), halo="auto", upstream: float = 1.0,
                                            out: Optional[torch.Tensor] = None) -> Tuple[torch.Tensor, torch.Tensor]:
        job = _voxel_multi_job(self, directions, pad, halo, None, "variance_voxel_multi_value_and_grad")
        vox32 = _check_voxel(self, voxel)
        lib = _hip.require_gpu()
        H, W = self.image_size
        T, K, dev = int(vox32.shape[0]), len(job.shifts), self.device
        if out is not None and (tuple(out.shape) != (T, 2, H, W) or out.dtype != torch.float32 or out.device != dev
                                or not out.is_contiguous()):
            raise ValueError(f"out must be a contiguous float32 tensor of shape {(T, 2, H, W)} on {dev}")
        iwes = _launch_iwe_voxel_multi(self, vox32, job)
        variances, moments = _image_variances(iwes, bool(omit_boundary))
        up = torch.full((K,), float(upstream) / K, dtype=torch.float32, device=dev)
        affine = torch.empty((K, 2), dtype=torch.float32, device=dev)
        with _hip.on_device(dev):
            check(lib.ebos_image_variance_affine_f32(ptr(moments), ptr(up), K, ptr(affine), stream_ptr()), "ebos_image_variance_affine")
        d_voxel = _launch_voxel_multi_bwd(self, vox32, job, iwes, affine, int(bool(omit_boundary)), out)
        return variances.mean(), d_voxel


INT32_MAX = 2 ** 31 - 1


class TimeAwarePlanStack(object):

    def __init__(self, plans: Sequence[EventPlan]):
        plans = list(plans)
        if not plans:
            raise ValueError("stack_time_aware: no plans")
        if len(plans) > _hip.CMAX_VOXEL_MAX_BATCH:
            raise ValueError(f"stack_time_aware: {len(plans)} plans, the batched kernels take at most {_hip.CMAX_VOXEL_MAX_BATCH}")
        first = plans[0]
        for b, plan in enumerate(plans):
            if not plan.binned or plan.x is None:
                raise ValueError(f"stack_time_aware: plan {b} is un-binned or lean; build it with emit='full', tile=..., time_bin=T")
            if plan.bins is None or plan.time_bin is None:
                raise ValueError(f"stack_time_aware: plan {b} holds no time bins (EventPlan.build(..., time_bin=T))")
            if plan.__dict__.get("_deferred"):
                raise ValueError(f"stack_time_aware: plan {b} is deferred (its build was not read back)")
            for what in ("image_size", "tile", "time_bin", "dt_bound"):
                a, v = getattr(first, what), getattr(plan, what)
                if (tuple(a) if isinstance(a, (tuple, list)) else a) != (tuple(v) if isinstance(v, (tuple, list)) else v):
                    name = "warp direction (dt_bound)" if what == "dt_bound" else what
                    raise ValueError(f"stack_time_aware: plan {b} differs from plan 0 in {name}: {v!r} against {a!r}")
            if plan.device != first.device:
                raise ValueError(f"stack_time_aware: plan {b} is on {plan.device}, plan 0 on {first.device}")
        self.ns = [int(p.n) for p in plans]
        if sum(self.ns) > INT32_MAX:
            raise ValueError(f"stack_time_aware: {sum(self.ns)} events in total are more than INT32_MAX")
        self.plans = plans
        self.image_size, self.tile, self.time_bin, self.dt_bound = first.image_size, tuple(first.tile), first.time_bin, first.dt_bound
        self.ref_fraction, self.normalized_t = first.ref_fraction, first.normalized_t
        self.n = sum(self.ns)
        if len(plans) == 1:
            self.x, self.y, self.dt, self.bins = (getattr(first, k)[:first.n] for k in ("x", "y", "dt", "bins"))
            self.key_offsets = first.key_offsets.to(torch.int32).contiguous()[None]
        else:
            self.x, self.y, self.dt = (torch.cat([getattr(p, k)[:p.n] for p in plans]).contiguous() for k in ("x", "y", "dt"))
            self.bins = torch.cat([p.bins[:p.n] for p in plans]).contiguous()
            bases = torch.tensor([sum(self.ns[:b]) for b in range(len(plans))], dtype=torch.int32, device=first.device)
            self.key_offsets = (torch.stack([p.key_offsets for p in plans]) + bases[:, None]).to(torch.int32).contiguous()

    @classmethod
    def from_raw(cls, cols: Sequence[torch.Tensor], ranges: Sequence[Tuple[int, int]], image_size: Tuple[int, int],
                 direction: Union[str, float], tile: Tuple[int, int], time_bin: int, roi=None, remove=None,
                 ticks_per_second: float = 1e6, normalize_t: bool = True) -> "TimeAwarePlanStack":
        if isinstance(tile, str):
            if tile != "auto":
                raise ValueError("tile must be a (tile_h, tile_w) pair or 'auto'")
            tile = choose_tile(image_size)
        if tile is None:
            raise ValueError("TimeAwarePlanStack.from_raw builds binned plans: tile must be a (tile_h, tile_w) pair or 'auto'")
        time_bin = ops.check_time_bins(time_bin)
        cols = tuple(cols)
        if len(cols) not in (3, 4):
            raise ValueError("cols must be (col, row, t) or (col, row, t, pol)")
        col, row, t = cols[:3]
        for name, v, dts in (("col", col, (torch.int16,)), ("row", row, (torch.int16,)), ("t", t, (torch.int32, torch.int64))):
            if not isinstance(v, torch.Tensor) or v.dim() != 1 or v.dtype not in dts:
                raise ValueError(f"TimeAwarePlanStack.from_raw: {name} must be a 1-D tensor, dtype in {dts}; "
                                 f"got {tuple(getattr(v, 'shape', ()))} {getattr(v, 'dtype', type(v).__name__)}")
        n_total = int(t.shape[0])
        if int(col.shape[0]) != n_total or int(row.shape[0]) != n_total:
            raise ValueError("TimeAwarePlanStack.from_raw: the raw columns must be of equal length")
        ranges = [(int(b), int(e)) for b, e in ranges]
        if not ranges:
            raise ValueError("TimeAwarePlanStack.from_raw: no windows")
        if len(ranges) > _hip.CMAX_VOXEL_MAX_BATCH:
            raise ValueError(f"TimeAwarePlanStack.from_raw: {len(ranges)} windows, the batched kernels take at most {_hip.CMAX_VOXEL_MAX_BATCH}")
        for b, e in ranges:
            if not 0 <= b <= e <= n_total:
                raise IndexError(f"TimeAwarePlanStack.from_raw: range [{b}, {e}) outside the {n_total} events")
        total = sum(e - b for b, e in ranges)
        if total > INT32_MAX:
            raise ValueError(f"TimeAwarePlanStack.from_raw: {total} events in total are more than INT32_MAX")
        rects = []
        for name, r in (("roi", roi), ("remove", remove)):
            if r is not None:
                r = tuple(r[k] for k in ("xmin", "xmax", "ymin", "ymax")) if isinstance(r, dict) else tuple(r)
                if len(r) != 4 or any(int(v) != v for v in r):
                    raise ValueError(f"{name} must be four integers (xmin, xmax, ymin, ymax), got {r!r}")
                r = tuple(int(v) for v in r)
                if r[0] > r[1] or r[2] > r[3]:
                    raise ValueError(f"{name} must have xmin <= xmax and ymin <= ymax, got {r!r}")
            rects.append(r)
        roi, remove = rects
        H, W = int(image_size[0]), int(image_size[1])
        th, tw = int(tile[0]), int(tile[1])
        if not (0 < H <= 32767 and 0 < W <= 32767 and th > 0 and tw > 0):
            raise ValueError(f"TimeAwarePlanStack.from_raw: bad image size {H} x {W} or tile {th} x {tw}")
        ref_mode, frac = parse_direction(direction)
        lib = _hip.require_gpu()
        for name, v in (("col", col), ("row", row), ("t", t)):
            if not v.is_cuda:
                raise _hip.HipUnavailableError(f"TimeAwarePlanStack.from_raw: {name} must be on the GPU")
        col, row, t = col.contiguous(), row.contiguous(), t.contiguous()
        dev, B = t.device, len(ranges)
        n_keys = ((H + th - 1) // th) * ((W + tw - 1) // tw) * th * tw
        c_ranges = (C.c_int64 * (2 * B))(*[v for r in ranges for v in r])
        nbytes = int(lib.ebos_plan_time_aware_batch_scratch_bytes(c_ranges, B, H, W, th, tw))
        if nbytes == 0:
            raise ValueError(f"TimeAwarePlanStack.from_raw: bad geometry: {B} windows of {H} x {W}, tile {th} x {tw}")
        scratch = torch.empty(nbytes, dtype=torch.uint8, device=dev)
        x, y, dt = (torch.zeros(total + 8, dtype=torch.float32, device=dev) for _ in range(3))
        bins = torch.zeros(total + 8, dtype=torch.uint8, device=dev)
        perm = torch.zeros(total + 8, dtype=torch.int32, device=dev)
        key_local = torch.empty((B, n_keys + 1), dtype=torch.int32, device=dev)
        key_stacked = torch.empty((B, n_keys + 1), dtype=torch.int32, device=dev)
        counts = torch.empty((B, 2), dtype=torch.int32, device=dev)
        tminmax = torch.empty((B, 2), dtype=torch.float64, device=dev)
        r4, m4 = roi or (0, 0, 0, 0), remove or (0, 0, 0, 0)
        with _hip.on_device(dev):
            check(lib.ebos_plan_time_aware_raw_batch(ptr(col), ptr(row), ptr(t), int(t.dtype == torch.int64), float(ticks_per_second),
                                                     n_total, c_ranges, B, int(roi is not None), *r4, int(remove is not None), *m4,
                                                     ref_mode, frac, int(bool(normalize_t)), time_bin, H, W, th, tw, ptr(x), ptr(y),
                                                     ptr(dt), ptr(bins), ptr(perm), total, ptr(key_local), ptr(key_stacked), n_keys + 1,
                                                     ptr(counts), ptr(tminmax), ptr(scratch), nbytes, stream_ptr()),
                  "ebos_plan_time_aware_raw_batch")
        host = counts.tolist()
        self = object.__new__(cls)
        self.ns = [int(c[0]) for c in host]
        self.n = sum(self.ns)
        self.image_size, self.tile, self.time_bin = (H, W), (th, tw), time_bin
        self.dt_bound = dt_bound_for(direction, normalize_t)
        self.ref_fraction, self.normalized_t = ref_fraction_for(direction), bool(normalize_t)
        self.x, self.y, self.dt, self.bins, self.perm = x[:self.n], y[:self.n], dt[:self.n], bins[:self.n], perm[:self.n]
        self.key_offsets, self.tminmax = key_stacked, tminmax
        self.plans, base = [], 0
        for b, (n, dropped) in enumerate(host):
            plan = EventPlan(x[base:base + n], y[base:base + n], dt[base:base + n], None, (H, W), n, n + dropped, (th, tw), key_local[b],
                             perm[base:base + n], dropped, dt_bound=self.dt_bound, bins=bins[base:base + n], time_bin=time_bin,
                             ref_fraction=self.ref_fraction, normalized_t=self.normalized_t)
            plan.__dict__["_frac"], plan.__dict__["_frac_pending"] = None, False
            plan.__dict__["_counts"], plan.__dict__["_deferred"] = None, False
            plan.__dict__["_parts_used"], plan.__dict__["_fullest_tile"] = None, None
            self.plans.append(plan)
            base += n
        return self

    def __len__(self) -> int:
        return len(self.plans)

    @property
    def device(self) -> torch.device:
        return self.key_offsets.device

    def canonical(self) -> "TimeAwarePlanStack":
        cached = self.__dict__.get("_canonical")
        if cached is None and len(self.plans) == 1:
            cached = self.__dict__["_canonical"] = self.plans[0].__dict__.get("_canonical_stack")
        if cached is None:
            cached = self.__dict__["_canonical"] = object.__new__(type(self))
            cached.__dict__.update({k: v for k, v in self.__dict__.items() if k not in ("_canonical", "perm")})
            if self.n > 0:
                n = self.n
                x, y, dt, bins = self.x[:n], self.y[:n], self.dt[:n], self.bins[:n]
                run = torch.searchsorted(self.key_offsets.reshape(-1).to(torch.int64), torch.arange(n, device=x.device), right=True)
                order = torch.arange(n, device=x.device)
                for key in (bins, y, x, dt, run):
                    order = order[torch.sort(key[order], stable=True)[1]]
                cached.x, cached.y, cached.dt, cached.bins = (v[order].contiguous() for v in (x, y, dt, bins))
            cached.__dict__["_canonical"] = cached
            if len(self.plans) == 1:
                self.plans[0].__dict__["_canonical_stack"] = cached
        return cached

    def ns_array(self):
        return (C.c_int64 * len(self.ns))(*self.ns)


def _build_lean(source: int, events, raw, image_size, direction, normalize_t, tile, ticks_per_second, deferred):
    lib = _hip.require_gpu()
    H, W = int(image_size[0]), int(image_size[1])
    th, tw = int(tile[0]), int(tile[1])
    if th > 256 or tw > 256:
        return None
    ref_mode, frac = parse_direction(direction)
    if raw is None:
        dev, n = events.device, int(events.shape[0])
        col = row = t = None
    else:
        col, row, t = raw
        dev, n = t.device, int(t.shape[0])
    tiles_y, tiles_x = (H + th - 1) // th, (W + tw - 1) // tw
    n_tiles, n_keys = tiles_y * tiles_x, tiles_y * tiles_x * th * tw
    nbytes = int(lib.ebos_plan_lean_scratch_bytes(n, H, W, th, tw))
    scratch = torch.empty(nbytes, dtype=torch.uint8, device=dev)
    cap = n + 3 * n_tiles + 8
    key_offsets = torch.empty(n_keys + 1, dtype=torch.int32, device=dev)
    grp_offsets = torch.empty(n_tiles + 1, dtype=torch.int32, device=dev)
    cpix = torch.empty(cap, dtype=torch.int16, device=dev)
    cdt = torch.empty(cap, dtype=torch.float32, device=dev)
    counts = torch.empty(2, dtype=torch.int32, device=dev)
    part_table = torch.empty(5 * n_tiles + 1, dtype=torch.int32, device=dev)
    with _hip.on_device(dev):
        rc = lib.ebos_plan_lean(source, ptr(events), ptr(col), ptr(row), ptr(t), float(ticks_per_second), n, ref_mode, frac,
                                int(normalize_t), H, W, th, tw, ptr(key_offsets), ptr(grp_offsets), ptr(cpix), ptr(cdt), cap,
                                ptr(counts), None, ptr(scratch), nbytes, stream_ptr())
        if rc == -3:
            return None
        check(rc, "ebos_plan_lean")
        check(lib.ebos_plan_parts(ptr(key_offsets), H, W, th, tw, _n_cu(dev), part_fixed_events(n, n_tiles, _n_cu(dev)), ptr(part_table),
                                  stream_ptr()), "ebos_plan_parts")
    dropped, used, fullest = 0, None, None
    if not deferred:
        dropped, fractional, used, fullest = _plan_facts(lib, key_offsets, H, W, th, tw, counts, part_table)
        if fractional:
            return None
    plan = EventPlan(None, None, None, None, (H, W), n - dropped, n, (th, tw), key_offsets, None, dropped, grp_offsets, cpix, cdt,
                     part_table, dt_bound_for(direction, normalize_t), ref_fraction=ref_fraction_for(direction),
                     normalized_t=bool(normalize_t))
    plan.__dict__["_counts"], plan.__dict__["_deferred"], plan.__dict__["_parts_used"] = counts, bool(deferred), used
    plan.__dict__["_fullest_tile"] = fullest
    return plan


def _plan_facts(lib, key_offsets: torch.Tensor, H: int, W: int, th: int, tw: int, counts: torch.Tensor, part_table: torch.Tensor):
    facts = torch.empty(4, dtype=torch.int32, device=key_offsets.device)
    with _hip.on_device(key_offsets.device):
        check(lib.ebos_plan_facts(ptr(key_offsets), H, W, th, tw, ptr(counts), ptr(part_table), ptr(facts), stream_ptr()), "ebos_plan_facts")
    return tuple(int(v) for v in facts.tolist())


def _check_flow(plan: EventPlan, flow: torch.Tensor) -> torch.Tensor:
    H, W = plan.image_size
    if tuple(flow.shape) != (2, H, W):
        raise ValueError(f"flow must be [2, {H}, {W}], got {tuple(flow.shape)}")
    if flow.device != plan.device:
        raise _hip.HipUnavailableError(f"flow is on {flow.device}, the event plan on {plan.device}")
    return flow.to(torch.float32).contiguous()


_SLAB_CONFIGS = None


def _slab_ok(plan: EventPlan, halo) -> bool:
    global _SLAB_CONFIGS
    if not plan.binned or halo is None:
        return False
    if _SLAB_CONFIGS is None:
        _SLAB_CONFIGS = set(_hip.slab_configs())
    if halo == "auto":
        return any((th, tw) == tuple(plan.tile) for th, tw, _ in _SLAB_CONFIGS)
    return (plan.tile[0], plan.tile[1], _max_halo(int(halo))) in _SLAB_CONFIGS


def _refuse_deferred(plan: EventPlan, what: str) -> None:
    if plan.__dict__.get("_deferred"):
        raise NotImplementedError(f"{what}: a plan built with deferred=True only runs on the tile-private kernels "
                                  "(a built tile / halo configuration); rebuild it with deferred=False for the general path")
    if plan.lean:
        raise NotImplementedError(f"{what}: a lean plan (emit='compact') holds no SoA events: it only runs on the tile-private "
                                  "kernels (a built tile / halo configuration) with unit weights; build it with emit='full'")


def _workspace(plan: EventPlan, pad, halo, splits) -> torch.Tensor:
    lib = _hip.require_gpu()
    key = (int(halo), int(splits), int(pad[0]), int(pad[1]))
    cache = plan.__dict__.setdefault("_workspaces", {})
    if key not in cache:
        H, W = plan.image_size
        nbytes = int(lib.ebos_iwe_slab_workspace_bytes(H, W, plan.tile[0], plan.tile[1], key[0], key[1], key[2], key[3]))
        cache[key] = torch.zeros(nbytes, dtype=torch.uint8, device=plan.device)
    return cache[key]


class SlabBatch(object):

    def __init__(self, plans, flows, patch=None, pad=(0, 0), halo: int = DEFAULT_HALO, splits: Optional[int] = None,
                 omit_boundary: bool = False):
        lib = _hip.require_gpu()
        if not plans:
            raise ValueError("SlabBatch: no windows")
        p0 = plans[0]
        H, W = p0.image_size
        self.plans, self.flows = list(plans), [f.contiguous().float() for f in flows]
        if halo == "auto":
            bounds = [pl.dt_bound for pl in plans]
            if any(b is None for b in bounds):
                halo = max(hl for th, tw, hl in _hip.slab_configs() if (th, tw) == tuple(p0.tile))
            else:
                halo = int(lib.ebos_halo_auto(max(hl for th, tw, hl in _hip.slab_configs() if (th, tw) == tuple(p0.tile)), float(max(bounds))))
        self.pad, self.halo, self.omit = (int(pad[0]), int(pad[1])), int(halo), bool(omit_boundary)
        self.splits = p0.resolve_splits(splits)
        for pl, fl in zip(self.plans, self.flows):
            if pl.image_size != p0.image_size or pl.tile != p0.tile or not pl.compact or pl.device != p0.device:
                raise ValueError("SlabBatch: windows must share image size, tile and device, and be compact (unit-weight) plans")
            if pl.resolve_splits(splits) != self.splits:
                raise ValueError("SlabBatch: windows must share the work-item mode (all adaptive or all with the same split count)")
        if patch is None:
            self.grid = (0, 0, 0, 0, 0, 0)
            want = (2, H, W)
        else:
            (ph, pw), (sh, sw) = patch
            gh, gw = self.flows[0].shape[-2:]
            self.grid = (int(gh), int(gw), int(ph), int(pw), int(sh), int(sw))
            want = (2, gh, gw)
        for fl in self.flows:
            if tuple(fl.shape) != want:
                raise ValueError(f"SlabBatch: flow of shape {tuple(fl.shape)}, expected {want}")
        n = len(self.plans)
        dev = p0.device
        self.nws = int(lib.ebos_iwe_slab_workspace_bytes(H, W, p0.tile[0], p0.tile[1], self.halo, self.splits, *self.pad))
        self.workspaces = torch.zeros((n, (self.nws + 255) // 256 * 256), dtype=torch.uint8, device=dev)
        self.iwes = torch.empty((n, H + 2 * self.pad[0], W + 2 * self.pad[1]), dtype=torch.float32, device=dev)
        self.variances = torch.empty(n, dtype=torch.float32, device=dev)
        self.moments = torch.empty((n, 2), dtype=torch.float64, device=dev)
        self.windows = (_hip.SlabWindow * n)()
        P = lambda t: None if t is None else t.data_ptr()
        for k, (pl, fl) in enumerate(zip(self.plans, self.flows)):
            w = self.windows[k]
            cp = pl._compact_ptrs()
            w.grp_offsets, w.cpix, w.cdt = cp[0], cp[1], cp[2]
            w.key_offsets, w.part_table, w.flow = P(pl.key_offsets), P(pl.part_table) if self.splits == 0 else None, P(fl)
            w.workspace, w.iwe = self.workspaces[k].data_ptr(), self.iwes[k].data_ptr()
            w.out_variance, w.moments = self.variances.data_ptr() + 4 * k, self.moments[k].data_ptr()
        self._lib, self._tile, self._size = lib, p0.tile, (H, W)

    def run(self, want_variance: bool = True, stream: Optional[int] = None, tail_stream: Optional[int] = None) -> torch.Tensor:
        H, W = self._size
        _hip.check(self._lib.ebos_iwe_slab_batch_f32(self.windows, len(self.plans), *self.grid, H, W, self._tile[0], self._tile[1],
                                                     self.halo, self.splits, self.pad[0], self.pad[1], self.workspaces.shape[1],
                                                     1 if want_variance else 0, 1 if self.omit else 0,
                                                     _hip.stream_ptr() if stream is None else stream, tail_stream),
                   "ebos_iwe_slab_batch")
        return self.variances


class _DenseJob(object):

    def __init__(self, plan: EventPlan, pad, halo, splits, omit):
        import ctypes as C

        H, W = plan.image_size
        self.ws = _workspace(plan, pad, halo, splits)
        self.iwe = torch.empty((H + 2 * pad[0], W + 2 * pad[1]), dtype=torch.float32, device=plan.device)
        self.moments = torch.empty((1, 2), dtype=torch.float64, device=plan.device)
        g, c, d = plan._compact_ptrs()
        self.struct = _hip.DenseJob(ptr(plan.x), ptr(plan.y), ptr(plan.dt), g, c, d, ptr(plan.key_offsets), plan.n, H, W,
                                    plan.tile[0], plan.tile[1], int(halo), int(splits), pad[0], pad[1], int(omit), ptr(self.ws),
                                    self.ws.numel(), ptr(plan.part_table), ptr(self.iwe), ptr(self.moments))
        self.ref = C.addressof(self.struct)
        self.index = plan.device.index
        self._gm = None

    def gm_buffers(self):
        if self._gm is None:
            lib = _hip.require_gpu()
            h, w = self.iwe.shape
            n = int(lib.ebos_gradient_magnitude_fused_partials(h, w))
            self._gm = (torch.empty_like(self.iwe), torch.empty(n, dtype=torch.float64, device=self.iwe.device), n)
        return self._gm


def _dense_job(plan: EventPlan, pad, halo, splits, omit) -> _DenseJob:
    key = ("job", int(pad[0]), int(pad[1]), int(halo), int(splits), bool(omit))
    cache = plan.__dict__.setdefault("_jobs", {})
    job = cache.get(key)
    if job is None:
        job = cache[key] = _DenseJob(plan, pad, halo, splits, omit)
    return job


_SIGNS = {}


def _sign_constant(device: torch.device, sign: float) -> torch.Tensor:
    key = (device, float(sign))
    t = _SIGNS.get(key)
    if t is None:
        t = _SIGNS[key] = torch.full((1,), float(sign), dtype=torch.float32, device=device)
    return t


def _run_dense_job(job: _DenseJob, flow32: torch.Tensor, want_grad: bool, cost: str = "image_variance", sign: float = 1.0):
    lib = _hip.require_gpu()
    out = torch.empty(2, dtype=torch.float32, device=flow32.device)
    d_flow = torch.empty_like(flow32) if want_grad else None
    up = None if sign == 1.0 else _sign_constant(flow32.device, sign).data_ptr()
    scaled = out.data_ptr() + 4 if want_grad else None

    def call():
        if cost == "image_variance":
            return lib.ebos_variance_dense_job_signed_f32(job.ref, flow32.data_ptr(), out.data_ptr(), scaled, up, ptr(d_flow), stream_ptr())
        d_iwe, partials, n = job.gm_buffers()
        return lib.ebos_gradient_magnitude_dense_job_f32(job.ref, flow32.data_ptr(), out.data_ptr(), scaled, up, ptr(d_flow),
                                                         d_iwe.data_ptr(), partials.data_ptr(), n, stream_ptr())

    if _hip.current_device_index() == job.index:
        rc = call()
    else:
        with _hip.on_device(flow32.device):
            rc = call()
    check(rc, "ebos_variance_dense_job" if cost == "image_variance" else "ebos_gradient_magnitude_dense_job")
    return out, d_flow


def _launch_iwe_dense_slab(plan: EventPlan, flow32, weight, pad, halo, splits, want_variance=False, omit=False):
    lib = _hip.require_gpu()
    H, W = plan.image_size
    ws = _workspace(plan, pad, halo, splits)
    iwe = torch.empty((H + 2 * pad[0], W + 2 * pad[1]), dtype=torch.float32, device=plan.device)
    out = torch.empty(1, dtype=torch.float32, device=plan.device) if want_variance else None
    moments = torch.empty((1, 2), dtype=torch.float64, device=plan.device) if want_variance else None
    with _hip.on_device(plan.device):
        check(lib.ebos_iwe_dense_slab_f32(ptr(plan.x), ptr(plan.y), ptr(plan.dt), ptr(weight), *plan._compact_ptrs(),
                                          ptr(plan.key_offsets), plan.n,
                                          ptr(flow32), H, W, plan.tile[0], plan.tile[1], int(halo), int(splits), pad[0],
                                          pad[1], ptr(ws), ws.numel(), ptr(iwe), int(want_variance), int(omit), ptr(out),
                                          ptr(moments), ptr(plan.part_table), stream_ptr()), "ebos_iwe_dense_slab")
    return iwe, out, moments


def _launch_iwe_dense(plan: EventPlan, flow32: torch.Tensor, weight, pad, halo, splits) -> torch.Tensor:
    lib = _hip.require_gpu()
    H, W = plan.image_size
    if _slab_ok(plan, halo):
        return _launch_iwe_dense_slab(plan, flow32, weight, pad, halo, splits)[0]
    _refuse_deferred(plan, "iwe_dense")
    iwe = torch.zeros((H + 2 * pad[0], W + 2 * pad[1]), dtype=torch.float32, device=plan.device)
    with _hip.on_device(plan.device):
        if plan.binned and halo is not None:
            check(lib.ebos_iwe_dense_tiled_f32(ptr(plan.x), ptr(plan.y), ptr(plan.dt), ptr(weight), ptr(plan.key_offsets),
                                               plan.n, ptr(flow32), H, W, plan.tile[0], plan.tile[1], int(halo), max(1, splits),
                                               pad[0], pad[1], ptr(iwe), stream_ptr()), "ebos_iwe_dense_tiled")
        else:
            check(lib.ebos_iwe_dense_f32(ptr(plan.x), ptr(plan.y), ptr(plan.dt), ptr(weight), plan.n, ptr(flow32), H, W,
                                         W, pad[0], pad[1], ptr(iwe), stream_ptr()), "ebos_iwe_dense")
    return iwe


def _plan_weight(plan: EventPlan, weight: Optional[torch.Tensor]) -> Optional[torch.Tensor]:
    if weight is None:
        return None
    if plan.__dict__.get("_deferred"):
        raise NotImplementedError("per-event weights need a plan built with the host read-back (deferred=False)")
    if plan.lean:
        raise NotImplementedError("per-event weights need the SoA events and the permutation: build the plan with emit='full'")
    w = weight.to(device=plan.device, dtype=torch.float32).reshape(-1)
    if w.numel() != plan.n_input:
        raise ValueError(f"weight must have one entry per input event ({plan.n_input}), got {w.numel()}")
    w = w if plan.perm is None else w[plan.perm.long()]
    out = torch.zeros((plan.n + 3) // 4 * 4 + 4, dtype=torch.float32, device=plan.device)
    out[:plan.n] = w
    return out[:plan.n]


def _launch_dense_bwd(plan, flow32, weight_p, pad, g_image, affine, g_lo, want_dweight, halo=DEFAULT_HALO,
                      var_moments=None, upstream=None, splits=1):
    lib = _hip.require_gpu()
    H, W = plan.image_size
    d_w = torch.empty(plan.n, dtype=torch.float32, device=plan.device) if want_dweight else None
    if _slab_ok(plan, halo):
        d_flow = torch.empty((2, H, W), dtype=torch.float32, device=plan.device)
        adaptive = splits == 0 and plan.part_table is not None
        ws = _workspace(plan, pad, halo, 0) if adaptive else None
        with _hip.on_device(plan.device):
            check(lib.ebos_iwe_dense_tiled_bwd_f32(ptr(plan.x), ptr(plan.y), ptr(plan.dt), ptr(weight_p), *plan._compact_ptrs(),
                                                   ptr(plan.key_offsets), plan.n, ptr(flow32), H, W, plan.tile[0], plan.tile[1], int(halo), pad[0],
                                                   pad[1], ptr(g_image), ptr(affine), g_lo, ptr(d_flow), ptr(d_w),
                                                   ptr(var_moments), ptr(upstream), None, ptr(ws), ws.numel() if adaptive else 0,
                                                   ptr(plan.part_table) if adaptive else None, stream_ptr()),
                  "ebos_iwe_dense_tiled_bwd")
        return d_flow, d_w
    _refuse_deferred(plan, "iwe_dense backward")
    if var_moments is not None:
        affine = torch.empty(2, dtype=torch.float32, device=plan.device)
        with _hip.on_device(plan.device):
            check(lib.ebos_image_variance_affine_f32(ptr(var_moments), ptr(upstream), 1, ptr(affine), stream_ptr()),
                  "ebos_image_variance_affine")
    d_flow = torch.zeros((2, H, W), dtype=torch.float32, device=plan.device)
    with _hip.on_device(plan.device):
        check(lib.ebos_iwe_dense_bwd_f32(ptr(plan.x), ptr(plan.y), ptr(plan.dt), ptr(weight_p), plan.n, ptr(flow32), H, W,
                                         W, pad[0], pad[1], ptr(g_image), ptr(affine), g_lo, int(plan.binned),
                                         ptr(d_flow), ptr(d_w), stream_ptr()), "ebos_iwe_dense_bwd")
    return d_flow, d_w


def _unpermute(plan: EventPlan, d_w: torch.Tensor) -> torch.Tensor:
    out = torch.zeros(plan.n_input, dtype=d_w.dtype, device=d_w.device)
    if plan.perm is None:
        out.copy_(d_w)
    else:
        out[plan.perm.long()] = d_w
    return out


class _FusedIweDense(torch.autograd.Function):
    @staticmethod
    def forward(ctx, flow, weight, plan, pad, halo, splits):
        flow32 = _check_flow(plan, flow)
        wp = _plan_weight(plan, weight)
        iwe = _launch_iwe_dense(plan, flow32, wp, pad, halo, splits)
        ctx.save_for_backward(flow32, wp if wp is not None else torch.empty(0))
        ctx.meta = (plan, pad, flow.dtype, weight.dtype if weight is not None else None, halo, splits)
        return iwe if flow.dtype == torch.float32 else iwe.to(flow.dtype)

    @staticmethod
    def backward(ctx, g):
        flow32, wp = ctx.saved_tensors
        plan, pad, fdt, wdt, halo, splits = ctx.meta
        wp = wp if wdt is not None else None
        need_w = wdt is not None and ctx.needs_input_grad[1]
        d_flow, d_w = _launch_dense_bwd(plan, flow32, wp, pad, g.to(torch.float32).contiguous(), None, 0, need_w, halo,
                                        splits=splits)
        d_weight = _unpermute(plan, d_w).to(wdt) if need_w else None
        return (d_flow.to(fdt) if ctx.needs_input_grad[0] else None), d_weight, None, None, None, None


MULTIREF_MAX = _hip.MULTIREF_MAX
MULTIREF_DEFAULT_FUSED = False


def multi_reference_fractions(directions) -> List[float]:
    if isinstance(directions, (str, float, int)) or directions is None:
        raise ValueError(f"directions must be a list of 1 to {MULTIREF_MAX} reference times, got {directions!r}")
# ... 710 lines not shown
```

include/ebos_hip.h:

```cpp
#ifndef EBOS_HIP_H
#define EBOS_HIP_H

#include <stddef.h>
#include <stdint.h>

#ifdef __cplusplus
extern "C" {
#endif

#define EBOS_ABI_VERSION 2

typedef void* ebos_stream_t;

typedef enum ebos_status {
  EBOS_OK = 0,
  EBOS_ERR_INVALID_ARG = -1,
  EBOS_ERR_LAUNCH = -2,
  EBOS_ERR_UNSUPPORTED = -3,
  EBOS_ERR_SCRATCH = -4
} ebos_status;

typedef enum ebos_reftime_mode {
  EBOS_REF_FIRST = 0,
  EBOS_REF_LAST = 1,
  EBOS_REF_FRACTION = 2,
  EBOS_REF_TIMEBASE = 3
} ebos_reftime_mode;

typedef enum ebos_splat_mode {
  EBOS_SPLAT_BILINEAR = 0,
  EBOS_SPLAT_COUNT = 1,
  EBOS_SPLAT_POLARITY = 2
} ebos_splat_mode;

int ebos_profile_start(int max_records);
int ebos_profile_stop(float* ms, int cap);
typedef enum ebos_profile_kernel {
  EBOS_PROFILE_SLAB_ACCUMULATE = 0,
  EBOS_PROFILE_TILED_BWD = 1,
  EBOS_PROFILE_SLAB_COMBINE = 2,
  EBOS_PROFILE_GRADMAG_FUSED = 3
} ebos_profile_kernel;
int ebos_profile_start_kernel(int which, int max_records);

int ebos_version(void);
const char* ebos_last_error(void);
const char* ebos_build_info(void);

int ebos_time_range_f32(const float* events, int64_t b, int64_t n, float* tminmax, ebos_stream_t stream);
int ebos_time_range_f64(const double* events, int64_t b, int64_t n, double* tminmax, ebos_stream_t stream);

int ebos_warp_dense_f32(const float* events, const float* flow, const float* tminmax, int ref_mode,
                        double ref_fraction, int normalize_t, int64_t b, int64_t n, int H, int W,
                        int row_stride, float* warped, int32_t* oob_count, ebos_stream_t stream);
int ebos_warp_dense_f64(const double* events, const double* flow, const double* tminmax, int ref_mode,
                        double ref_fraction, int normalize_t, int64_t b, int64_t n, int H, int W,
                        int row_stride, double* warped, int32_t* oob_count, ebos_stream_t stream);

int ebos_warp_dense_bwd_f32(const float* events, const float* tminmax, int ref_mode, double ref_fraction,
                            int normalize_t, const float* d_warped, int64_t b, int64_t n, int H, int W,
                            int row_stride, float* d_flow, ebos_stream_t stream);
int ebos_warp_dense_bwd_f64(const double* events, const double* tminmax, int ref_mode, double ref_fraction,
                            int normalize_t, const double* d_warped, int64_t b, int64_t n, int H, int W,
                            int row_stride, double* d_flow, ebos_stream_t stream);

int ebos_warp_2dof_f32(const float* events, const float* theta, const float* tminmax, int ref_mode,
                       double ref_fraction, int normalize_t, const float* time_period, int64_t n,
                       float* warped, ebos_stream_t stream);
int ebos_warp_2dof_f64(const double* events, const double* theta, const double* tminmax, int ref_mode,
                       double ref_fraction, int normalize_t, const double* time_period, int64_t n,
                       double* warped, ebos_stream_t stream);
int ebos_warp_2dof_bwd_f32(const float* events, const float* tminmax, int ref_mode, double ref_fraction,
                           int normalize_t, const float* time_period, const float* d_warped, int64_t n,
                           float* d_theta, ebos_stream_t stream);
int ebos_warp_2dof_bwd_f64(const double* events, const double* tminmax, int ref_mode, double ref_fraction,
                           int normalize_t, const double* time_period, const double* d_warped, int64_t n,
                           double* d_theta, ebos_stream_t stream);

int ebos_splat_f32(const float* events, const float* weight, double weight_scalar, int mode, double eps,
                   int64_t b, int64_t n, int h, int w, int pad_h, int pad_w, float* image,
                   ebos_stream_t stream);
int ebos_splat_f64(const double* events, const double* weight, double weight_scalar, int mode, double eps,
                   int64_t b, int64_t n, int h, int w, int pad_h, int pad_w, double* image,
                   ebos_stream_t stream);

int ebos_splat_bwd_f32(const float* events, const float* weight, double weight_scalar, double eps,
                       const float* d_image, int64_t b, int64_t n, int h, int w, int pad_h, int pad_w,
                       float* d_events, float* d_weight, ebos_stream_t stream);
int ebos_splat_bwd_f64(const double* events, const double* weight, double weight_scalar, double eps,
                       const double* d_image, int64_t b, int64_t n, int h, int w, int pad_h, int pad_w,
                       double* d_events, double* d_weight, ebos_stream_t stream);

int ebos_events_to_soa_f32(const float* events, const float* tminmax, int ref_mode, double ref_fraction,
                           int normalize_t, int64_t n, float* x, float* y, float* dt, float* p,
                           ebos_stream_t stream);
int ebos_events_to_soa_f64(const double* events, const double* tminmax, int ref_mode, double ref_fraction,
                           int normalize_t, int64_t n, float* x, float* y, float* dt, float* p,
                           ebos_stream_t stream);

int ebos_raw_time_range(const void* t, int t_bytes, int64_t n, double ticks_per_second, int64_t* scratch_ticks,
                        double* tminmax, ebos_stream_t stream);
int ebos_raw_events_to_soa(const int16_t* col, const int16_t* row, const void* t, int t_bytes,
                           const uint8_t* pol, double ticks_per_second, const double* tminmax, int ref_mode,
                           double ref_fraction, int normalize_t, int64_t n, float* x, float* y, float* dt,
                           float* p, ebos_stream_t stream);

size_t ebos_bin_scratch_bytes(int64_t n_keys);
size_t ebos_bin_scratch_bytes_events(int64_t n, int H, int W, int tile_h, int tile_w);
int ebos_bin_events_f32(const float* x, const float* y, const float* dt, const float* p, int64_t n,
                        int H, int W, int tile_h, int tile_w, float* xs, float* ys, float* dts, float* ps,
                        int32_t* perm, int32_t* key_offsets, int32_t* oob_count, int32_t* frac_count,
                        void* scratch, size_t scratch_bytes, ebos_stream_t stream);

int ebos_plan_parts(const int32_t* key_offsets, int H, int W, int tile_h, int tile_w, int n_cu, int fixed_events,
                    int32_t* part_table, ebos_stream_t stream);

int ebos_plan_facts(const int32_t* key_offsets, int H, int W, int tile_h, int tile_w, const int32_t* counts,
                    const int32_t* part_table, int32_t* facts, ebos_stream_t stream);

size_t ebos_plan_lean_scratch_bytes(int64_t n, int H, int W, int tile_h, int tile_w);
int ebos_plan_lean(int source, const void* events, const int16_t* col, const int16_t* row, const void* t,
                   double ticks_per_second, int64_t n, int ref_mode, double ref_fraction, int normalize_t, int H, int W,
                   int tile_h, int tile_w, int32_t* key_offsets, int32_t* grp_offsets, uint16_t* cpix, float* cdt,
                   int64_t capacity_slots, int32_t* counts, double* tminmax, void* scratch, size_t scratch_bytes,
                   ebos_stream_t stream);
size_t ebos_plan_lean_batch_scratch_bytes(const int64_t* ranges, int n_windows, int H, int W, int tile_h, int tile_w);
int ebos_plan_lean_batch(const int16_t* col, const int16_t* row, const void* t, int t_is_64, double ticks_per_second, int64_t n_total,
                         const int64_t* ranges, int n_windows, int ref_mode, double ref_fraction, int normalize_t, int H, int W,
                         int tile_h, int tile_w, int32_t* key_offsets, int64_t key_stride, int32_t* grp_offsets, int64_t grp_stride,
                         uint16_t* cpix, float* cdt, const int64_t* slot_offsets, int32_t* counts, double* tminmax, void* scratch,
                         size_t scratch_bytes, ebos_stream_t stream);
int ebos_plan_parts_batch(const int32_t* key_offsets, int64_t key_stride, int n_windows, int H, int W, int tile_h, int tile_w, int n_cu,
                          const int32_t* fixed_events, int32_t* part_table, int64_t part_stride, ebos_stream_t stream);
int ebos_plan_facts_batch(const int32_t* key_offsets, int64_t key_stride, int n_windows, int H, int W, int tile_h, int tile_w,
                          const int32_t* counts, const int32_t* part_table, int64_t part_stride, int32_t* facts, ebos_stream_t stream);
int ebos_plan_compact_f32(const float* xs, const float* ys, const float* dts, const int32_t* key_offsets, int64_t n,
                          int H, int W, int tile_h, int tile_w, int32_t* grp_offsets, uint16_t* cpix, float* cdt,
                          int64_t capacity_slots, ebos_stream_t stream);
int ebos_plan_compact_frac_f32(const float* xs, const float* ys, const float* dts, const int32_t* key_offsets, int64_t n,
                               int H, int W, int tile_h, int tile_w, int32_t* grp_offsets, uint16_t* cpix, float* cdt,
                               float* cfx, float* cfy, int64_t capacity_slots, ebos_stream_t stream);

int ebos_iwe_dense_f32(const float* x, const float* y, const float* dt, const float* weight, int64_t n,
                       const float* flow, int H, int W, int row_stride, int pad_h, int pad_w, float* iwe,
                       ebos_stream_t stream);
int ebos_iwe_dense_tiled_f32(const float* xs, const float* ys, const float* dts, const float* weight,
                             const int32_t* key_offsets, int64_t n, const float* flow, int H, int W,
                             int tile_h, int tile_w, int halo, int splits, int pad_h, int pad_w,
                             float* iwe, ebos_stream_t stream);
int ebos_tiled_config(int* out, int cap);

int ebos_iwe_dense_bwd_f32(const float* x, const float* y, const float* dt, const float* weight, int64_t n,
                           const float* flow, int H, int W, int row_stride, int pad_h, int pad_w,
                           const float* g_image, const float* affine, int g_lo, int sorted, float* d_flow,
                           float* d_weight, ebos_stream_t stream);

#define EBOS_HALO_AUTO(max_halo, dt_bound_q64) (-((int)(max_halo) + 256 * (int)(dt_bound_q64)))
int ebos_halo_auto(int max_halo, double dt_bound);
int ebos_slab_config(int* out, int cap);
size_t ebos_iwe_slab_workspace_bytes(int H, int W, int tile_h, int tile_w, int halo, int splits, int pad_h,
                                     int pad_w);
int ebos_iwe_slab_partials(int H, int W, int tile_h, int tile_w, int halo, int splits, int pad_h, int pad_w,
                           int omit_boundary, size_t* offset_bytes, int64_t* n_partials, int64_t* n_pixels);
int ebos_iwe_dense_slab_f32(const float* xs, const float* ys, const float* dts, const float* weight,
                            const int32_t* grp_offsets, const uint16_t* cpix, const float* cdt,
                            const int32_t* key_offsets, int64_t n, const float* flow, int H, int W, int tile_h,
                            int tile_w, int halo, int splits, int pad_h, int pad_w, void* workspace,
                            size_t workspace_bytes, float* iwe, int want_variance, int omit_boundary,
                            float* out_variance, double* moments, const int32_t* part_table,
                            ebos_stream_t stream);
typedef struct ebos_dense_job {
  const float *xs, *ys, *dts;
  const int32_t* grp_offsets;
  const uint16_t* cpix;
  const float* cdt;
  const int32_t* key_offsets;
  int64_t n;
  int H, W, tile_h, tile_w, halo, splits, pad_h, pad_w, omit_boundary;
  void* workspace;
  size_t workspace_bytes;
  const int32_t* part_table;
  float* iwe;
  double* moments;
} ebos_dense_job;
int ebos_variance_dense_job_f32(const ebos_dense_job* job, const float* flow, float* out_variance, const float* upstream,
                                float* d_flow, ebos_stream_t stream);
int ebos_gradient_magnitude_dense_job_f32(const ebos_dense_job* job, const float* flow, float* out_contrast, float* out_scaled,
                                          const float* upstream, float* d_flow, float* d_iwe, double* partials, int64_t n_partials,
                                          ebos_stream_t stream);
int ebos_variance_dense_job_signed_f32(const ebos_dense_job* job, const float* flow, float* out_variance, float* out_scaled,
                                       const float* upstream, float* d_flow, ebos_stream_t stream);
int ebos_iwe_dense_tiled_bwd_f32(const float* xs, const float* ys, const float* dts, const float* weight,
                                 const int32_t* grp_offsets, const uint16_t* cpix, const float* cdt,
                                 const int32_t* key_offsets, int64_t n, const float* flow, int H, int W,
                                 int tile_h, int tile_w, int halo, int pad_h, int pad_w, const float* g_image,
                                 const float* affine, int g_lo, float* d_flow, float* d_weight,
                                 const double* var_moments, const float* upstream, const float* addend,
                                 void* workspace, size_t workspace_bytes, const int32_t* part_table,
                                 ebos_stream_t stream);

int ebos_patch_fused_supported(int tile_h, int tile_w, int halo, int slide_h, int slide_w);
typedef struct ebos_slab_window {
  const int32_t* grp_offsets;
  const uint16_t* cpix;
  const float* cdt;
  const int32_t* key_offsets;
  const int32_t* part_table;
  const float* flow;
  void* workspace;
  float* iwe;
  float* out_variance;
  double* moments;
} ebos_slab_window;
int ebos_iwe_slab_batch_f32(const ebos_slab_window* windows, int n_windows, int gh, int gw, int patch_h, int patch_w, int slide_h,
                            int slide_w, int H, int W, int tile_h, int tile_w, int halo, int splits, int pad_h, int pad_w,
                            size_t workspace_bytes, int want_variance, int omit_boundary, ebos_stream_t stream,
                            ebos_stream_t tail_stream);

int ebos_iwe_patch_slab_f32(const int32_t* grp_offsets, const uint16_t* cpix, const float* cdt,
                            const int32_t* key_offsets, int64_t n, const float* grid, int gh, int gw, int patch_h,
                            int patch_w, int slide_h, int slide_w, int H, int W, int tile_h, int tile_w, int halo,
                            int splits, int pad_h, int pad_w, void* workspace, size_t workspace_bytes, float* iwe,
                            int want_variance, int omit_boundary, float* out_variance, double* moments,
                            const int32_t* part_table, ebos_stream_t stream);
int ebos_iwe_patch_slab_frac_f32(const int32_t* grp_offsets, const uint16_t* cpix, const float* cdt, const float* cfx, const float* cfy,
                                 const int32_t* key_offsets, int64_t n, const float* grid, int gh, int gw, int patch_h, int patch_w,
                                 int slide_h, int slide_w, int H, int W, int tile_h, int tile_w, int halo, int splits, int pad_h,
                                 int pad_w, void* workspace, size_t workspace_bytes, float* iwe, int want_variance, int omit_boundary,
                                 float* out_variance, double* moments, const int32_t* part_table, ebos_stream_t stream);
size_t ebos_patch_grad_partials_bytes(int H, int W, int tile_h, int tile_w, int adaptive);
int ebos_iwe_patch_tiled_bwd_f32(const int32_t* grp_offsets, const uint16_t* cpix, const float* cdt,
                                 const int32_t* key_offsets, int64_t n, const float* grid, int gh, int gw,
                                 int patch_h, int patch_w, int slide_h, int slide_w, int H, int W, int tile_h,
                                 int tile_w, int halo, int pad_h, int pad_w, const float* g_image,
                                 const float* affine, int g_lo, const double* var_moments, const float* upstream,
                                 const float* addend, float* grad_partials, size_t grad_partials_bytes,
                                 const int32_t* part_table, float w_flow_norm, float w_image_gradient,
                                 double* reg_partials,
                                 const double* var_partials, int64_t n_var_partials, int64_t n_var_pixels,
                                 float* out_variance, double* out_moments, ebos_stream_t stream);
int ebos_iwe_patch_tiled_bwd_blur_f32(const int32_t* grp_offsets, const uint16_t* cpix, const float* cdt,
                                      const int32_t* key_offsets, int64_t n, const float* grid, int gh, int gw,
                                      int patch_h, int patch_w, int slide_h, int slide_w, int H, int W, int tile_h,
                                      int tile_w, int halo, int pad_h, int pad_w, const float* z_image, int g_lo,
                                      const float* upstream, float* grad_partials, size_t grad_partials_bytes,
                                      const int32_t* part_table, float w_flow_norm, float w_image_gradient,
                                      double* reg_partials, const double* blur_partials, int64_t n_blur_partials,
                                      int64_t n_var_pixels, float* out_variance, double* out_moments, float blur_k0,
                                      float blur_k1, ebos_stream_t stream);
int ebos_iwe_patch_tiled_bwd_frac_f32(const int32_t* grp_offsets, const uint16_t* cpix, const float* cdt, const float* cfx, const float* cfy,
                                      const int32_t* key_offsets, int64_t n, const float* grid, int gh, int gw, int patch_h, int patch_w,
                                      int slide_h, int slide_w, int H, int W, int tile_h, int tile_w, int halo, int pad_h, int pad_w,
                                      const float* g_image, int g_lo, const double* var_moments, const float* upstream,
                                      const float* addend, float* grad_partials, size_t grad_partials_bytes, const int32_t* part_table,
                                      float w_flow_norm, float w_image_gradient, double* reg_partials, const double* var_partials,
                                      int64_t n_var_partials, int64_t n_var_pixels, float* out_variance, double* out_moments,
                                      float blur_k0, float blur_k1, ebos_stream_t stream);
int ebos_iwe_dense_tiled_bwd_blur_f32(const float* xs, const float* ys, const float* dts, const int32_t* grp_offsets, const uint16_t* cpix,
                                      const float* cdt, const int32_t* key_offsets, int64_t n, const float* flow, int H, int W, int tile_h,
                                      int tile_w, int halo, int pad_h, int pad_w, const float* z_image, int g_lo, const float* upstream,
                                      const float* addend, float* d_flow, void* workspace, size_t workspace_bytes,
                                      const int32_t* part_table, const double* blur_partials, int64_t n_blur_partials,
                                      int64_t n_var_pixels, float* out_variance, double* out_moments, float blur_k0, float blur_k1,
                                      ebos_stream_t stream);
int ebos_patch_grad_combine_adam_f32(const float* grad_partials, const int32_t* part_table, int tile_h, int tile_w,
                                     int gh, int gw, int patch_h, int patch_w, int slide_h, int slide_w, int H, int W,
                                     float* d_grid, float* theta, float* exp_avg, float* exp_avg_sq, double lr,
                                     double beta1, double beta2, double eps, int t, int* step, const float* contrast,
                                     float contrast_scale, const double* reg_partials, int n_reg, float* losses,
                                     int losses_cap, const float* grad_mask, ebos_stream_t stream);

int ebos_iwe_2dof_slab_f32(const float* xs, const float* ys, const float* dts, const float* weight,
                           const int32_t* grp_offsets, const uint16_t* cpix, const float* cdt,
                           const int32_t* key_offsets, int64_t n, const float* thetas, int K,
                           int H, int W, int tile_h, int tile_w, int halo, int splits, int pad_h, int pad_w,
                           void* workspace, size_t workspace_bytes, float* iwes, int want_variance,
                           int omit_boundary, float* out_variance, double* moments, const int32_t* part_table,
                           ebos_stream_t stream);

int ebos_iwe_2dof_slab_batch_f32(const int32_t* grp_offsets, const uint16_t* cpix, const float* cdt,
                                 const int32_t* key_offsets, int64_t n, const float* thetas, int K, int H, int W,
                                 int tile_h, int tile_w, int halo, int splits, int pad_h, int pad_w, void* workspaces,
                                 size_t workspace_bytes, float* iwes, int want_variance, int omit_boundary,
                                 float* out_variance, double* moments, const int32_t* part_table, ebos_stream_t stream,
                                 ebos_stream_t tail_stream);

int ebos_iwe_2dof_tiled_bwd_f32(const float* xs, const float* ys, const float* dts, const float* weight,
                                const int32_t* grp_offsets, const uint16_t* cpix, const float* cdt,
                                const int32_t* key_offsets, int64_t n, const float* thetas,
                                int K, int H, int W, int tile_h, int tile_w, int halo, int pad_h, int pad_w,
                                const float* g_images, const float* affine, int g_lo, float* d_thetas,
                                void* workspace, size_t workspace_bytes, ebos_stream_t stream);

int ebos_iwe_2dof_f32(const float* x, const float* y, const float* dt, const float* weight, int64_t n,
                      const float* thetas, int K, int h, int w, int pad_h, int pad_w, float* iwes,
                      ebos_stream_t stream);
int ebos_iwe_2dof_bwd_f32(const float* x, const float* y, const float* dt, const float* weight, int64_t n,
                          const float* thetas, int K, int h, int w, int pad_h, int pad_w,
                          const float* g_images, const float* affine, int g_lo, float* d_thetas,
                          ebos_stream_t stream);

size_t ebos_cost_scratch_bytes(int K);
int ebos_image_variance_f32(const float* images, int K, int h, int w, int omit_boundary, float* out,
                            double* moments, void* scratch, size_t scratch_bytes, ebos_stream_t stream);
int ebos_image_variance_grad_f32(const float* images, int K, int h, int w, int omit_boundary,
                                 const double* moments, const float* upstream, float* d_images,
                                 ebos_stream_t stream);
int ebos_image_variance_affine_f32(const double* moments, const float* upstream, int K, float* affine,
                                   ebos_stream_t stream);
int ebos_gradient_magnitude_f32(const float* images, int K, int h, int w, int omit_boundary, float* out,
                                void* scratch, size_t scratch_bytes, ebos_stream_t stream);
int ebos_gradient_magnitude_grad_f32(const float* images, int K, int h, int w, int omit_boundary,
                                     const float* upstream, float* d_images, ebos_stream_t stream);
int ebos_image_variance_f64(const double* images, int K, int h, int w, int omit_boundary, double* out,
                            double* moments, void* scratch, size_t scratch_bytes, ebos_stream_t stream);
int ebos_image_variance_grad_f64(const double* images, int K, int h, int w, int omit_boundary,
                                 const double* moments, const double* upstream, double* d_images,
                                 ebos_stream_t stream);
int ebos_gradient_magnitude_f64(const double* images, int K, int h, int w, int omit_boundary, double* out,
                                void* scratch, size_t scratch_bytes, ebos_stream_t stream);
int ebos_gradient_magnitude_grad_f64(const double* images, int K, int h, int w, int omit_boundary,
                                     const double* upstream, double* d_images, ebos_stream_t stream);
int64_t ebos_gradient_magnitude_fused_partials(int h, int w);
int ebos_gradient_magnitude_fused_f32(const float* image, int h, int w, int omit_boundary, const float* upstream, float* out,
                                      float* d_image, double* partials, int64_t n_partials, ebos_stream_t stream);

int64_t ebos_blur3_variance_partials(int h, int w);
size_t ebos_cmax_cost_scratch_bytes(int h, int w);
int ebos_blur3_variance_adjoint_f32(const float* image, int h, int w, int omit_boundary, float k0, float k1, float* z_image,
                                    double* partials, int64_t n_partials, ebos_stream_t stream);

int ebos_upsample_patch_flow_f32(const float* grid, int gh, int gw, int patch_h, int patch_w, int slide_h,
                                 int slide_w, int H, int W, float* dense, ebos_stream_t stream);
size_t ebos_upsample_bwd_scratch_bytes(int gh, int W);
int ebos_upsample_patch_flow_bwd_f32(const float* d_dense, int gh, int gw, int patch_h, int patch_w,
                                     int slide_h, int slide_w, int H, int W, float* scratch, float* d_grid,
                                     ebos_stream_t stream);
int ebos_upsample_patch_flow_bwd_adam_f32(const float* d_dense, int gh, int gw, int patch_h, int patch_w,
                                          int slide_h, int slide_w, int H, int W, float* scratch, float* d_grid,
                                          float* theta, float* exp_avg, float* exp_avg_sq, double lr, double beta1,
                                          double beta2, double eps, int t, int* step, const float* contrast,
                                          float contrast_scale, const double* reg_partials, int n_reg, float* losses,
                                          int losses_cap, const float* grad_mask, ebos_stream_t stream);

int ebos_gauss1d_f32(const float* in, float* out, int64_t outer, int64_t L, int64_t inner, const double* taps,
                     int radius, int boundary, ebos_stream_t stream);
int ebos_gauss1d_f64(const double* in, double* out, int64_t outer, int64_t L, int64_t inner, const double* taps,
                     int radius, int boundary, ebos_stream_t stream);
int ebos_gauss1d_bwd_f32(const float* g_out, float* g_in, int64_t outer, int64_t L, int64_t inner,
                         const double* taps, int radius, int boundary, ebos_stream_t stream);
int ebos_gauss1d_bwd_f64(const double* g_out, double* g_in, int64_t outer, int64_t L, int64_t inner,
                         const double* taps, int radius, int boundary, ebos_stream_t stream);

int ebos_flow_regularisers_partials(void);
int ebos_flow_regularisers_f32(const float* flow, int H, int W, float w_flow_norm, float w_image_gradient,
                               float* d_flow, double* partials, const double* var_partials, int64_t n_var_partials,
                               int64_t n_var_pixels, float* out_variance, double* moments, ebos_stream_t stream);
int ebos_cmax_adam_step_f32(float* theta, const float* grad, float* exp_avg, float* exp_avg_sq, int n, double lr,
                            double beta1, double beta2, double eps, int* step, const float* contrast,
                            float contrast_scale, const double* reg_partials, int n_reg, float* losses,
                            int losses_cap, ebos_stream_t stream);

typedef struct ebos_cmax_patch_problem {
  const float *xs, *ys, *dts;
  const int32_t* grp_offsets;
  const uint16_t* cpix;
  const float* cdt;
  const int32_t* key_offsets;
  int64_t n;
  int H, W, tile_h, tile_w, halo, pad_h, pad_w, omit_boundary;
  int splits;
  const int32_t* part_table;
  int gh, gw, patch_h, patch_w, slide_h, slide_w;
  float w_variance, w_flow_norm, w_image_gradient;
  float w_gradient_magnitude;
  double lr, beta1, beta2, eps;
  float *theta, *d_theta, *exp_avg, *exp_avg_sq;
  int* step;
  int steps_done;
  float *dense, *d_dense, *d_reg, *iwe, *variance;
  float* d_iwe;
  void* cost_scratch;
  size_t cost_scratch_bytes;
  double* moments;
  const float* upstream;
  double* reg_partials;
  float* upsample_scratch;
  void* workspace;
  size_t workspace_bytes;
  float* losses;
  int losses_cap;
  const float* theta_mask;
  float* grad_partials;
  size_t grad_partials_bytes;
  float blur_k0, blur_k1;
  float* blur_image;
  const float *cfx, *cfy;
} ebos_cmax_patch_problem;
int ebos_cmax_patch_solve_f32(const ebos_cmax_patch_problem* problem, int n_iter, ebos_stream_t stream);
int ebos_cmax_patch_gradient_f32(const ebos_cmax_patch_problem* problem, ebos_stream_t stream);
int ebos_cmax_patch_solve_many_f32(const ebos_cmax_patch_problem* problems, const ebos_stream_t* streams,
                                   int n_problems, int n_iter);

typedef struct ebos_cmax_2dof_problem {
  const float *xs, *ys, *dts;
  const int32_t* grp_offsets;
  const uint16_t* cpix;
  const float* cdt;
  const float *cfx, *cfy;
  const int32_t* key_offsets;
  int64_t n;
  int H, W, tile_h, tile_w, halo, pad_h, pad_w, omit_boundary;
  int splits;
  const int32_t* part_table;
  float w_variance;
  float blur_k0, blur_k1;
  double lr, beta1, beta2, eps;
  float *theta, *d_theta, *exp_avg, *exp_avg_sq;
  int* step;
  int steps_done;
  float *iwe, *blur_image, *variance;
  double* moments;
// ... 502 lines not shown
```

Before: 387,600.

## Compute event dt in staging pass assuming sorted window, verify and fall back

When the sorted-window hint is set, the staging kernel reads the first and last event timestamps, builds the time reference from them, and writes the final float dt packed with the pixel as one 8-byte record. This lets the bin sort load finished dt values instead of raw stamps plus a separate pixel array. The totals kernel checks that the true min and max match those edges and that no NaN was seen, and reports whether the window was sorted. If not, the Python side reruns the whole plan without the hint, so unsorted inputs pay for two passes and an extra host sync through tolist.

Result: no change. 388,400 (median of 4 runs) (+0.2%).

```diff
diff --git a/event_based_bos_amd/csrc/plan_lean.hip b/event_based_bos_amd/csrc/plan_lean.hip
--- a/event_based_bos_amd/csrc/plan_lean.hip
+++ b/event_based_bos_amd/csrc/plan_lean.hip
@@ -25,6 +25,7 @@
 constexpr size_t kSortLds = 158 * 1024;
 
 enum LeanSource { SRC_AOS_F32 = 0, SRC_AOS_F64 = 1, SRC_RAW32 = 2, SRC_RAW64 = 3 };
+constexpr unsigned kLeanDoneSources = 0xF;
 
 struct LeanIn {
   const void* events;
@@ -140,6 +141,54 @@
   }
 }
 
+struct LeanTime {
+  int src, ref_mode, normalize_t;
+  double ref_fraction, ticks_per_second;
+};
+
+struct LeanRec {
+  unsigned pix;
+  unsigned long long stamp;
+};
+struct LeanDone {
+  unsigned pix;
+  float dt;
+};
+__device__ __forceinline__ LeanDone unpack_done(unsigned long long v) { return LeanDone{(unsigned)(v >> 32), __uint_as_float((unsigned)v)}; }
+struct LeanClock {
+  double ref, inv_period, tps;
+  bool raw, wide;
+  __device__ __forceinline__ LeanClock() : ref(0.0), inv_period(1.0), tps(1.0), raw(false), wide(false) {}
+  __device__ __forceinline__ LeanClock(double tmin, double tmax, const LeanTime& tc) {
+    raw = tc.src == SRC_RAW32 || tc.src == SRC_RAW64;
+    wide = tc.src == SRC_AOS_F64 || tc.src == SRC_RAW64;
+    tps = tc.ticks_per_second;
+    if (raw) {
+      tmin = tmin / tps;
+      tmax = tmax / tps;
+    } else if (tc.src == SRC_AOS_F32) {
+      tmin = (double)(float)tmin;
+      tmax = (double)(float)tmax;
+    }
+    if (tc.ref_mode == EBOS_REF_FIRST) ref = tmin;
+    else if (tc.ref_mode == EBOS_REF_LAST) ref = tmax;
+    else ref = tmin + (tmax - tmin) * tc.ref_fraction;
+    inv_period = tc.normalize_t ? 1.0 / (tmax - tmin) : 1.0;
+  }
+  __device__ __forceinline__ LeanClock(const LeanScratch& sc, const LeanTime& tc) : LeanClock(unordered(sc.tm[0]), unordered(sc.tm[1]), tc) {}
+  __device__ __forceinline__ float dt(const LeanRec& r) const {
+    const double t8 = raw ? (double)(long long)r.stamp / tps : __longlong_as_double((long long)r.stamp);
+    const double t4 = raw ? (double)(int32_t)(unsigned)r.stamp / tps : (double)__uint_as_float((unsigned)r.stamp);
+    return (float)(((wide ? t8 : t4) - ref) * inv_period);
+  }
+};
+__device__ __forceinline__ double wave_uniform(double v) {
+  const long long b = __double_as_longlong(v);
+  const unsigned lo = __builtin_amdgcn_readfirstlane((int)(unsigned)b), hi = __builtin_amdgcn_readfirstlane((int)(unsigned)((unsigned long long)b >> 32));
+  return __longlong_as_double((long long)(((unsigned long long)hi << 32) | lo));
+}
+constexpr int kTmEdge = 16;
+
 __device__ __forceinline__ int32_t block_exclusive_scan(int32_t v, int32_t* s_wave , int32_t& total) {
   const int lane = threadIdx.x & (kWave - 1), wid = threadIdx.x / kWave;
   int32_t inc = v;
@@ -167,18 +216,20 @@
   int64_t n;
   LeanGeom g;
   LeanScratch sc;
+  LeanTime tc;
   struct View {
     LeanIn in;
     int64_t n;
     LeanGeom g;
     LeanScratch sc;
+    LeanTime tc;
     __device__ __forceinline__ unsigned index() const { return blockIdx.x; }
     __device__ __forceinline__ unsigned count() const { return gridDim.x; }
   };
-  __device__ __forceinline__ View view() const { return View{in, n, g, sc}; }
-};
-
-template <int SRC, typename Args>
+  __device__ __forceinline__ View view() const { return View{in, n, g, sc, tc}; }
+};
+
+template <int SRC, typename Args, bool DONE = false>
 __global__ void __launch_bounds__(kLeanBlock, 8)
 lean_stage_kernel(Args args) {
   const typename Args::View v = args.view();
@@ -186,7 +237,8 @@
   const int64_t n = v.n;
   const LeanGeom g = v.g;
   const LeanScratch sc = v.sc;
-  typedef typename StageT<SRC>::type stamp_t;
+  typedef typename std::conditional<DONE, unsigned long long, typename StageT<SRC>::type>::type stamp_t;
+  typedef typename std::conditional<DONE, float, typename StageT<SRC>::type>::type held_t;
   extern __shared__ int32_t s_mem[];
   int32_t* s_hist = s_mem;
   stamp_t* s_t = reinterpret_cast<stamp_t*>(s_mem + ((g.n_bins + 1) & ~1));
@@ -203,7 +255,22 @@
   int bad = 0, frac = 0;
   int bin_of[kPer];
   unsigned pix[kPer];
-  stamp_t stamp[kPer];
+  held_t stamp[kPer];
+  LeanClock clock;
+  int nan = 0;
+  if constexpr (DONE) {
+    float ex, ey;
+    double edge0, edge1;
+    read_stamp<SRC>(in, 0, ex, ey, edge0);
+    read_stamp<SRC>(in, n - 1, ex, ey, edge1);
+    edge0 = wave_uniform(edge0);
+    edge1 = wave_uniform(edge1);
+    if (v.index() == 0 && threadIdx.x == 0) {
+      sc.tm[kTmEdge] = (unsigned long long)__double_as_longlong(edge0);
+      sc.tm[kTmEdge + 1] = (unsigned long long)__double_as_longlong(edge1);
+    }
+    clock = LeanClock(edge0, edge1, LeanTime{SRC, v.tc.ref_mode, v.tc.normalize_t, v.tc.ref_fraction, v.tc.ticks_per_second});
+  }
 #pragma unroll
   for (int k = 0; k < kPer; ++k) {
     if (k == kPer / 2) asm volatile("" ::: "memory");
@@ -212,7 +279,13 @@
     if (i < chunk_end) {
       float x, y;
       double t;
-      stamp[k] = read_stamp<SRC>(in, i, x, y, t);
+      const typename StageT<SRC>::type bits = read_stamp<SRC>(in, i, x, y, t);
+      if constexpr (DONE) {
+        stamp[k] = clock.dt(LeanRec{0u, (unsigned long long)bits});
+        nan |= t != t;
+      } else {
+        stamp[k] = bits;
+      }
       lo = t < lo ? t : lo;
       hi = t > hi ? t : hi;
       bool fr;
@@ -247,16 +320,22 @@
   for (int k = 0; k < kPer; ++k)
     if (bin_of[k] >= 0) {
       const int pos = s_hist[bin_of[k] & 8191] + (bin_of[k] >> 13);
-      s_t[pos] = stamp[k];
-      s_px[pos] = (uint16_t)pix[k];
+      if constexpr (DONE) {
+        reinterpret_cast<uint2*>(s_t)[pos] = make_uint2(__float_as_uint(stamp[k]), pix[k]);
+      } else {
+        s_t[pos] = stamp[k];
+        s_px[pos] = (uint16_t)pix[k];
+      }
     }
   __syncthreads();
   EBOS_LSTAMP(0, 4);
   stamp_t* out_t = static_cast<stamp_t*>(sc.stage_t) + base;
   for (int i = threadIdx.x; i < kept; i += kLeanBlock) out_t[i] = s_t[i];
-  unsigned* out_px = reinterpret_cast<unsigned*>(sc.stage_px + base);
-  const unsigned* s_px2 = reinterpret_cast<const unsigned*>(s_px);
-  for (int i = threadIdx.x; i < (kept + 1) / 2; i += kLeanBlock) out_px[i] = s_px2[i];
+  if constexpr (!DONE) {
+    unsigned* out_px = reinterpret_cast<unsigned*>(sc.stage_px + base);
+    const unsigned* s_px2 = reinterpret_cast<const unsigned*>(s_px);
+    for (int i = threadIdx.x; i < (kept + 1) / 2; i += kLeanBlock) out_px[i] = s_px2[i];
+  }
   __shared__ double s_lo[kLeanBlock / kWave], s_hi[kLeanBlock / kWave];
   __shared__ int s_bad[kLeanBlock / kWave], s_frac[kLeanBlock / kWave];
   lo = wave_min(lo);
@@ -269,7 +348,8 @@
     s_bad[threadIdx.x / kWave] = bad;
     s_frac[threadIdx.x / kWave] = frac;
   }
-  __syncthreads();
+  if constexpr (DONE) nan = __syncthreads_or(nan);
+  else __syncthreads();
   if (threadIdx.x == 0) {
     for (int k = 1; k < kLeanBlock / kWave; ++k) {
       lo = s_lo[k] < lo ? s_lo[k] : lo;
@@ -277,6 +357,7 @@
       bad += s_bad[k];
       frac += s_frac[k];
     }
+    if (DONE && nan) lo = __builtin_nan("");
     sc.partial[v.index()] = ChunkPartial{lo, hi, bad, frac};
   }
   EBOS_LSTAMP(0, 5);
@@ -347,7 +428,8 @@
 template <typename Grid>
 __device__ __forceinline__ void lean_totals_body(const LeanGeom& g, int n_chunks, const LeanScratch& sc, int32_t* __restrict__ counts,
                                                  int32_t* __restrict__ grp_offsets, int32_t* __restrict__ key_offsets, int64_t n_keys,
-                                                 double ticks_per_second, int raw, double* __restrict__ tminmax, const Grid grid) {
+                                                 double ticks_per_second, int raw, double* __restrict__ tminmax, const Grid grid,
+                                                 int32_t* __restrict__ sorted = nullptr, int edges = 0) {
   __shared__ int s_is_last;
   {
     const int bin = grid.index() * (kLeanBlock / kWave) + (int)(threadIdx.x / kWave), lane = threadIdx.x & (kWave - 1);
@@ -372,25 +454,28 @@
   }
   if (grid.index() == 0) {
     double lo = 1.0e308 * 10.0, hi = -1.0e308 * 10.0;
-    int bad = 0, frac = 0;
+    int bad = 0, frac = 0, nan = 0;
     for (int c = threadIdx.x; c < n_chunks; c += kLeanBlock) {
       const ChunkPartial p = sc.partial[c];
       lo = p.lo < lo ? p.lo : lo;
       hi = p.hi > hi ? p.hi : hi;
       bad += p.bad;
       frac += p.frac;
+      nan += p.lo != p.lo;
     }
     __shared__ double s_lo[kLeanBlock / kWave], s_hi[kLeanBlock / kWave];
-    __shared__ int s_bad[kLeanBlock / kWave], s_frac[kLeanBlock / kWave];
+    __shared__ int s_bad[kLeanBlock / kWave], s_frac[kLeanBlock / kWave], s_nan[kLeanBlock / kWave];
     lo = wave_min(lo);
     hi = wave_max(hi);
     bad = wave_sum(bad);
     frac = wave_sum(frac);
+    nan = wave_sum(nan);
     if ((threadIdx.x & (kWave - 1)) == 0) {
       s_lo[threadIdx.x / kWave] = lo;
       s_hi[threadIdx.x / kWave] = hi;
       s_bad[threadIdx.x / kWave] = bad;
       s_frac[threadIdx.x / kWave] = frac;
+      s_nan[threadIdx.x / kWave] = nan;
     }
     __syncthreads();
     if (threadIdx.x == 0) {
@@ -399,7 +484,11 @@
         hi = s_hi[k] > hi ? s_hi[k] : hi;
         bad += s_bad[k];
         frac += s_frac[k];
-      }
+        nan += s_nan[k];
+      }
+      if (sorted != nullptr)
+        *sorted = !edges || (nan == 0 && (unsigned long long)__double_as_longlong(lo) == sc.tm[kTmEdge] &&
+                             (unsigned long long)__double_as_longlong(hi) == sc.tm[kTmEdge + 1]);
       typedef __attribute__((address_space(1))) unsigned long long gu64_;
       __hip_atomic_store((gu64_*)&sc.tm[0], lo <= hi ? ordered(lo) : ~0ull, __ATOMIC_RELAXED, __HIP_MEMORY_SCOPE_AGENT);
       __hip_atomic_store((gu64_*)&sc.tm[1], lo <= hi ? ordered(hi) : 0ull, __ATOMIC_RELAXED, __HIP_MEMORY_SCOPE_AGENT);
@@ -427,14 +516,10 @@
 
 __global__ void __launch_bounds__(kLeanBlock)
 lean_totals_kernel(LeanGeom g, int n_chunks, LeanScratch sc, int32_t* __restrict__ counts, int32_t* __restrict__ grp_offsets,
-                   int32_t* __restrict__ key_offsets, int64_t n_keys, double ticks_per_second, int raw, double* __restrict__ tminmax) {
-  lean_totals_body(g, n_chunks, sc, counts, grp_offsets, key_offsets, n_keys, ticks_per_second, raw, tminmax, WholeGrid{});
-}
-
-struct LeanTime {
-  int src, ref_mode, normalize_t;
-  double ref_fraction, ticks_per_second;
-};
+                   int32_t* __restrict__ key_offsets, int64_t n_keys, double ticks_per_second, int raw, double* __restrict__ tminmax,
+                   int32_t* __restrict__ sorted, int edges) {
+  lean_totals_body(g, n_chunks, sc, counts, grp_offsets, key_offsets, n_keys, ticks_per_second, raw, tminmax, WholeGrid{}, sorted, edges);
+}
 
 template <int STRIDE>
 __device__ __forceinline__ int row_xor(int v) {
@@ -477,37 +562,6 @@
   const int b = __float_as_int(d);
   return b ^ ((b >> 31) & 0x7fffffff);
 }
-
-struct LeanRec {
-  unsigned pix;
-  unsigned long long stamp;
-};
-struct LeanClock {
-  double ref, inv_period, tps;
-  bool raw, wide;
-  __device__ __forceinline__ LeanClock(const LeanScratch& sc, const LeanTime& tc) {
-    raw = tc.src == SRC_RAW32 || tc.src == SRC_RAW64;
-    wide = tc.src == SRC_AOS_F64 || tc.src == SRC_RAW64;
-    tps = tc.ticks_per_second;
-    double tmin = unordered(sc.tm[0]), tmax = unordered(sc.tm[1]);
-    if (raw) {
-      tmin = tmin / tps;
-      tmax = tmax / tps;
-    } else if (tc.src == SRC_AOS_F32) {
-      tmin = (double)(float)tmin;
-      tmax = (double)(float)tmax;
-    }
-    if (tc.ref_mode == EBOS_REF_FIRST) ref = tmin;
-    else if (tc.ref_mode == EBOS_REF_LAST) ref = tmax;
-    else ref = tmin + (tmax - tmin) * tc.ref_fraction;
-    inv_period = tc.normalize_t ? 1.0 / (tmax - tmin) : 1.0;
-  }
-  __device__ __forceinline__ float dt(const LeanRec& r) const {
-    const double t8 = raw ? (double)(long long)r.stamp / tps : __longlong_as_double((long long)r.stamp);
-    const double t4 = raw ? (double)(int32_t)(unsigned)r.stamp / tps : (double)__uint_as_float((unsigned)r.stamp);
-    return (float)(((wide ? t8 : t4) - ref) * inv_period);
-  }
-};
 
 template <bool POS, int BLOCK, typename Load, typename Use>
 __device__ __forceinline__ void lean_gather(const LeanScratch& sc, const LeanGeom& g, int bin, int n_chunks, int32_t* s_arrived, Load&& load,
@@ -558,6 +612,7 @@
   }
 }
 
+template <bool DONE>
 __device__ __forceinline__ void lean_bin_sort_body(const LeanGeom& g, const LeanScratch& sc, const int32_t* __restrict__ grp_offsets,
                                                    int32_t* __restrict__ key_offsets, uint16_t* __restrict__ cpix, float* __restrict__ cdt,
                                                    int pix_cap, int sort_cap, int n_chunks, const LeanTime& tc) {
@@ -586,12 +641,17 @@
   __syncthreads();
   const bool staged = len <= sort_cap;
   const int lane = threadIdx.x & (kWave - 1);
-  const LeanClock clock(sc, tc);
-  typedef LeanRec Rec;
-  auto dt_of = [&](const Rec& r) { return clock.dt(r); };
+  LeanClock clock;
+  if constexpr (!DONE) clock = LeanClock(sc, tc);
+  typedef typename std::conditional<DONE, LeanDone, LeanRec>::type Rec;
+  auto dt_of = [&](const Rec& r) {
+    if constexpr (DONE) return r.dt;
+    else return clock.dt(r);
+  };
   const bool wide = clock.wide;
-  auto load8 = [&](int64_t i) { return Rec{(unsigned)sc.stage_px[i], static_cast<const unsigned long long*>(sc.stage_t)[i]}; };
-  auto load4 = [&](int64_t i) { return Rec{(unsigned)sc.stage_px[i], (unsigned long long)static_cast<const unsigned*>(sc.stage_t)[i]}; };
+  auto load_done = [&](int64_t i) { return unpack_done(static_cast<const unsigned long long*>(sc.stage_t)[i]); };
+  auto load8 = [&](int64_t i) { return LeanRec{(unsigned)sc.stage_px[i], static_cast<const unsigned long long*>(sc.stage_t)[i]}; };
+  auto load4 = [&](int64_t i) { return LeanRec{(unsigned)sc.stage_px[i], (unsigned long long)static_cast<const unsigned*>(sc.stage_t)[i]}; };
   auto for_each_staged = [&](auto with_pos, auto&& load, auto&& use) {
     lean_gather<decltype(with_pos)::value, kSortBlock>(sc, g, bin, n_chunks, &s_arrived, load, use);
   };
@@ -601,11 +661,16 @@
       a_dt[at] = dt_of(r);
       atomicAdd(&s_cnt[((int)(r.pix >> 8) - r0) * g.tw + (int)(r.pix & 255u)], 1);
     };
-    if (wide) for_each_staged(std::true_type{}, load8, arrive);
-    else for_each_staged(std::true_type{}, load4, arrive);
+    if constexpr (DONE) {
+      for_each_staged(std::true_type{}, load_done, arrive);
+    } else {
+      if (wide) for_each_staged(std::true_type{}, load8, arrive);
+      else for_each_staged(std::true_type{}, load4, arrive);
+    }
   } else {
-    for_each_staged(std::false_type{}, [&](int64_t i) { return (unsigned)sc.stage_px[i]; },
-                    [&](unsigned pix, int) { atomicAdd(&s_cnt[((int)(pix >> 8) - r0) * g.tw + (int)(pix & 255u)], 1); });
+    auto count = [&](unsigned pix, int) { atomicAdd(&s_cnt[((int)(pix >> 8) - r0) * g.tw + (int)(pix & 255u)], 1); };
+    if constexpr (DONE) for_each_staged(std::false_type{}, [&](int64_t i) { return static_cast<const unsigned*>(sc.stage_t)[2 * i + 1]; }, count);
+    else for_each_staged(std::false_type{}, [&](int64_t i) { return (unsigned)sc.stage_px[i]; }, count);
   }
   __syncthreads();
   EBOS_LSTAMP(1, 1);
@@ -686,8 +751,12 @@
           }
         }
       };
-      if (wide) for_each_staged(std::false_type{}, load8, keep);
-      else for_each_staged(std::false_type{}, load4, keep);
+      if constexpr (DONE) {
+        for_each_staged(std::false_type{}, load_done, keep);
+      } else {
+        if (wide) for_each_staged(std::false_type{}, load8, keep);
+        else for_each_staged(std::false_type{}, load4, keep);
+      }
       if (direct) {
         p_lo = p_hi;
         continue;
@@ -793,10 +862,11 @@
   }
 }
 
+template <bool DONE>
 __global__ void __launch_bounds__(kSortBlock)
 lean_bin_sort_kernel(LeanGeom g, LeanScratch sc, const int32_t* __restrict__ grp_offsets, int32_t* __restrict__ key_offsets,
                      uint16_t* __restrict__ cpix, float* __restrict__ cdt, int pix_cap, int sort_cap, int n_chunks, LeanTime tc) {
-  lean_bin_sort_body(g, sc, grp_offsets, key_offsets, cpix, cdt, pix_cap, sort_cap, n_chunks, tc);
+  lean_bin_sort_body<DONE>(g, sc, grp_offsets, key_offsets, cpix, cdt, pix_cap, sort_cap, n_chunks, tc);
 }
 
 struct LeanSections {
@@ -941,7 +1011,7 @@
   const int64_t wi = o.first + (int64_t)blockIdx.y;
   int pix_cap, sort_cap;
   lean_sort_caps(g.th, g.tw, g.sub, pix_cap, sort_cap);
-  lean_bin_sort_body(g, lean_window_scratch(o, g, w), o.grp_offsets + wi * o.grp_stride, o.key_offsets + wi * o.key_stride,
+  lean_bin_sort_body<false>(g, lean_window_scratch(o, g, w), o.grp_offsets + wi * o.grp_stride, o.key_offsets + wi * o.key_stride,
                      o.cpix + w.slot_off, o.cdt + w.slot_off, pix_cap, sort_cap, w.n_chunks, tc);
 }
 
@@ -966,6 +1036,8 @@
                    int32_t* key_offsets, int32_t* grp_offsets, uint16_t* cpix, float* cdt, int64_t capacity_slots, int32_t* counts,
                    double* tminmax, void* scratch, size_t scratch_bytes, ebos_stream_t stream) {
   using namespace ebos;
+  const bool ask_sorted = (source & EBOS_LEAN_SORTED_WINDOW) != 0;
+  source &= ~EBOS_LEAN_SORTED_WINDOW;
   EBOS_REQUIRE(source >= 0 && source <= 3, "ebos_plan_lean: source must be 0 (f32 [n,4]), 1 (f64 [n,4]), 2 (raw, int32 t), 3 (raw, int64 t)");
   EBOS_REQUIRE(n >= 1 && n < (int64_t)1 << 31, "ebos_plan_lean: 1 <= n < 2^31 (got %lld)", (long long)n);
   EBOS_REQUIRE(H > 0 && W > 0 && tile_h > 0 && tile_w > 0 && tile_h <= 256 && tile_w <= 256, "ebos_plan_lean: bad sizes (tiles up to 256 x 256)");
@@ -994,34 +1066,43 @@
   const LeanGeom g{H, W, tile_h, tile_w, tiles_x, n_tiles, L.sub, L.n_bins, L.chunk,
                    small ? (unsigned)(0x100000000ull / (unsigned)tile_h) + 1u : 0u, small ? (unsigned)(0x100000000ull / (unsigned)tile_w) + 1u : 0u};
   const LeanIn in{events, col, row, t, ticks_per_second};
+  const bool done = ask_sorted && ((kLeanDoneSources >> source) & 1u) != 0;
   const size_t stamp_bytes = (source == SRC_AOS_F64 || source == SRC_RAW64) ? 8 : 4;
-  const size_t lds_stage = (size_t)((L.n_bins + 1) & ~1) * 4 + (size_t)L.chunk * (stamp_bytes + 2);
+  const size_t lds_stage = (size_t)((L.n_bins + 1) & ~1) * 4 + (size_t)L.chunk * (done ? 8 : stamp_bytes + 2);
+  const LeanTime tc{source, ref_mode, normalize_t, ref_fraction, ticks_per_second};
   const size_t lds_sort = (size_t)(2 * L.pix_cap) * 4 + (size_t)L.sort_cap * 12;
-  bool ok = hipFuncSetAttribute(reinterpret_cast<const void*>(lean_bin_sort_kernel), hipFuncAttributeMaxDynamicSharedMemorySize,
-                                (int)kSortLds) == hipSuccess;
-#define EBOS_LEAN_ATTR(SRC)                                                                                                  \
-  ok = ok && hipFuncSetAttribute(reinterpret_cast<const void*>(lean_stage_kernel<SRC, StageOne>), hipFuncAttributeMaxDynamicSharedMemorySize, \
-                                 (int)lds_stage) == hipSuccess
-#define EBOS_LEAN(SRC)                                                                                                       \
-  do {                                                                                                                       \
-    EBOS_LEAN_ATTR(SRC);                                                                                                     \
-    if (ok) lean_stage_kernel<SRC, StageOne><<<dim3(L.n_chunks), dim3(kLeanBlock), lds_stage, s>>>(StageOne{in, n, g, sc});  \
+  const void* sort_fn = done ? reinterpret_cast<const void*>(lean_bin_sort_kernel<true>) : reinterpret_cast<const void*>(lean_bin_sort_kernel<false>);
+  bool ok = hipFuncSetAttribute(sort_fn, hipFuncAttributeMaxDynamicSharedMemorySize, (int)kSortLds) == hipSuccess;
+#define EBOS_LEAN_AS(SRC, DONE)                                                                                                        \
+  do {                                                                                                                                 \
+    ok = ok && hipFuncSetAttribute(reinterpret_cast<const void*>(lean_stage_kernel<SRC, StageOne, DONE>),                              \
+                                   hipFuncAttributeMaxDynamicSharedMemorySize, (int)lds_stage) == hipSuccess;                          \
+    if (ok) lean_stage_kernel<SRC, StageOne, DONE><<<dim3(L.n_chunks), dim3(kLeanBlock), lds_stage, s>>>(StageOne{in, n, g, sc, tc}); \
+  } while (0)
+#define EBOS_LEAN(SRC)                   \
+  do {                                   \
+    if (done) EBOS_LEAN_AS(SRC, true);   \
+    else EBOS_LEAN_AS(SRC, false);       \
   } while (0)
   if (source == SRC_AOS_F32) EBOS_LEAN(SRC_AOS_F32);
   else if (source == SRC_AOS_F64) EBOS_LEAN(SRC_AOS_F64);
   else if (source == SRC_RAW32) EBOS_LEAN(SRC_RAW32);
   else EBOS_LEAN(SRC_RAW64);
 #undef EBOS_LEAN
-#undef EBOS_LEAN_ATTR
+#undef EBOS_LEAN_AS
   if (!ok) {
     set_error("ebos_plan_lean: cannot reserve LDS for the staging pass / the bin sort");
     return EBOS_ERR_LAUNCH;
   }
   lean_totals_kernel<<<dim3((L.n_bins + kLeanBlock / kWave - 1) / (kLeanBlock / kWave)), dim3(kLeanBlock), 0, s>>>(g, L.n_chunks, sc, counts, grp_offsets, key_offsets, n_keys,
-                                                                                     ticks_per_second, source >= SRC_RAW32, tminmax);
-  const LeanTime tc{source, ref_mode, normalize_t, ref_fraction, ticks_per_second};
-  lean_bin_sort_kernel<<<dim3(8 * ((L.n_bins + 7) / 8)), dim3(kSortBlock), lds_sort, s>>>(g, sc, grp_offsets, key_offsets, cpix, cdt, L.pix_cap, L.sort_cap,
-                                                                          L.n_chunks, tc);
+                                                                                     ticks_per_second, source >= SRC_RAW32, tminmax,
+                                                                                     ask_sorted ? counts + 2 : nullptr, done ? 1 : 0);
+  if (done)
+    lean_bin_sort_kernel<true><<<dim3(8 * ((L.n_bins + 7) / 8)), dim3(kSortBlock), lds_sort, s>>>(g, sc, grp_offsets, key_offsets, cpix, cdt, L.pix_cap,
+                                                                                  L.sort_cap, L.n_chunks, tc);
+  else
+    lean_bin_sort_kernel<false><<<dim3(8 * ((L.n_bins + 7) / 8)), dim3(kSortBlock), lds_sort, s>>>(g, sc, grp_offsets, key_offsets, cpix, cdt, L.pix_cap,
+                                                                                   L.sort_cap, L.n_chunks, tc);
   EBOS_CHECK_LAUNCH("ebos_plan_lean");
   return EBOS_OK;
 }
diff --git a/event_based_bos_amd/event_plan.py b/event_based_bos_amd/event_plan.py
--- a/event_based_bos_amd/event_plan.py
+++ b/event_based_bos_amd/event_plan.py
@@ -1,6 +1,7 @@
 from __future__ import annotations
 
 import ctypes as C
+import os
 from dataclasses import dataclass, fields
 from typing import List, NamedTuple, Optional, Sequence, Tuple, Union
 
@@ -926,6 +927,9 @@
         return (C.c_int64 * len(self.ns))(*self.ns)
 
 
+_LEAN_SORTED_WINDOW = 0x100
+
+
 def _build_lean(source: int, events, raw, image_size, direction, normalize_t, tile, ticks_per_second, deferred):
     lib = _hip.require_gpu()
     H, W = int(image_size[0]), int(image_size[1])
@@ -948,27 +952,39 @@
     grp_offsets = torch.empty(n_tiles + 1, dtype=torch.int32, device=dev)
     cpix = torch.empty(cap, dtype=torch.int16, device=dev)
     cdt = torch.empty(cap, dtype=torch.float32, device=dev)
-    counts = torch.empty(2, dtype=torch.int32, device=dev)
+    back = torch.empty(8, dtype=torch.int32, device=dev)
+    counts = back[4:7]
     part_table = torch.empty(5 * n_tiles + 1, dtype=torch.int32, device=dev)
-    with _hip.on_device(dev):
-        rc = lib.ebos_plan_lean(source, ptr(events), ptr(col), ptr(row), ptr(t), float(ticks_per_second), n, ref_mode, frac,
-                                int(normalize_t), H, W, th, tw, ptr(key_offsets), ptr(grp_offsets), ptr(cpix), ptr(cdt), cap,
-                                ptr(counts), None, ptr(scratch), nbytes, stream_ptr())
-        if rc == -3:
-            return None
-        check(rc, "ebos_plan_lean")
-        check(lib.ebos_plan_parts(ptr(key_offsets), H, W, th, tw, _n_cu(dev), part_fixed_events(n, n_tiles, _n_cu(dev)), ptr(part_table),
-                                  stream_ptr()), "ebos_plan_parts")
-    dropped, used, fullest = 0, None, None
-    if not deferred:
-        dropped, fractional, used, fullest = _plan_facts(lib, key_offsets, H, W, th, tw, counts, part_table)
+    sorted_fast = not deferred and os.environ.get("EBOS_PLAN_SORTED_FAST", "1") != "0"
+    dropped, used, fullest, was_sorted = 0, None, None, None
+    for hint in ((_LEAN_SORTED_WINDOW, 0) if sorted_fast else (0,)):
+        with _hip.on_device(dev):
+            rc = lib.ebos_plan_lean(source | hint, ptr(events), ptr(col), ptr(row), ptr(t), float(ticks_per_second), n, ref_mode, frac,
+                                    int(normalize_t), H, W, th, tw, ptr(key_offsets), ptr(grp_offsets), ptr(cpix), ptr(cdt), cap,
+                                    ptr(counts), None, ptr(scratch), nbytes, stream_ptr())
+            if rc == -3:
+                return None
+            check(rc, "ebos_plan_lean")
+            check(lib.ebos_plan_parts(ptr(key_offsets), H, W, th, tw, _n_cu(dev), part_fixed_events(n, n_tiles, _n_cu(dev)), ptr(part_table),
+                                      stream_ptr()), "ebos_plan_parts")
+            if deferred:
+                break
+            check(lib.ebos_plan_facts(ptr(key_offsets), H, W, th, tw, ptr(counts), ptr(part_table), ptr(back), stream_ptr()), "ebos_plan_facts")
+        got = back.tolist()
+        dropped, fractional, used, fullest = got[:4]
         if fractional:
             return None
+        if not hint:
+            break
+        was_sorted = bool(got[6])
+        if was_sorted:
+            break
     plan = EventPlan(None, None, None, None, (H, W), n - dropped, n, (th, tw), key_offsets, None, dropped, grp_offsets, cpix, cdt,
                      part_table, dt_bound_for(direction, normalize_t), ref_fraction=ref_fraction_for(direction),
                      normalized_t=bool(normalize_t))
-    plan.__dict__["_counts"], plan.__dict__["_deferred"], plan.__dict__["_parts_used"] = counts, bool(deferred), used
+    plan.__dict__["_counts"], plan.__dict__["_deferred"], plan.__dict__["_parts_used"] = counts[:2], bool(deferred), used
     plan.__dict__["_fullest_tile"] = fullest
+    plan.__dict__["_sorted_window"] = was_sorted
     return plan
 
 
diff --git a/include/ebos_hip.h b/include/ebos_hip.h
--- a/include/ebos_hip.h
+++ b/include/ebos_hip.h
@@ -118,6 +118,7 @@
 int ebos_plan_facts(const int32_t* key_offsets, int H, int W, int tile_h, int tile_w, const int32_t* counts,
                     const int32_t* part_table, int32_t* facts, ebos_stream_t stream);
 
+#define EBOS_LEAN_SORTED_WINDOW 0x100
 size_t ebos_plan_lean_scratch_bytes(int64_t n, int H, int W, int tile_h, int tile_w);
 int ebos_plan_lean(int source, const void* events, const int16_t* col, const int16_t* row, const void* t,
                    double ticks_per_second, int64_t n, int ref_mode, double ref_fraction, int normalize_t, int H, int W,
```
